# VITA-Group/CV_A-FAN

Hardware: AMD Instinct MI355X
Metric: images/sec (whole node) A-FAN K=5 train step, ResNet-18/CIFAR-10 (higher is better)
Workload: dtype bf16; 1 GPU; resnet18 CIFAR-10-shape A-FAN K=5 bf16, batch 256/GPU, perturb_idx 6, internal layout nhwc, 1xMI355X per rank (BASELINE configs[1]); global_batch=256, parallelism=dp1, hipgraph=True, in_launch_batchnorm=True

## Files before the change

cv_a-fan_amd/_lib.py:

```python
import ctypes as C
import os

_HERE = os.path.dirname(os.path.abspath(__file__))
LIB_PATH = os.environ.get("AFAN_HIP_LIB") or os.path.join(_HERE, "libafan_hip.so")

AFAN_F32, AFAN_BF16 = 0, 1
AFAN_NCHW, AFAN_NHWC = 0, 1
_ERRORS = {-1: "AFAN_EDTYPE (unknown dtype code)", -2: "AFAN_EALIGN (misaligned pointer)",
           -3: "AFAN_ESHAPE (bad sizes)", -4: "AFAN_ENULL (required pointer is NULL)",
           -5: "AFAN_ELAYOUT (unknown layout code)"}

_p, _i, _l, _f = C.c_void_p, C.c_int, C.c_int64, C.c_float

SIGNATURES = {
    "afan_version": (_i, []),
    "afan_arch": (C.c_char_p, []),
    "afan_pgd_step": (_i, [_p, _p, _i, _p, _p, _l, _f, _f, _i, _p]),
    "afan_tensor_clamp": (_i, [_p, _p, _p, _l, _p]),
    "afan_norms_workspace_floats": (_l, [_l, _l]),
    "afan_pgd_step_norms": (_i, [_p, _p, _i, _p, _p, _l, _l, _f, _f, _i, _p, _p, _p, _p]),
    "afan_perturb_norms": (_i, [_p, _p, _l, _l, _p, _p, _p, _p]),
    "afan_axpy_noise": (_i, [_p, _p, _l, _f, _p, _p]),
    "afan_mix_feature": (_i, [_p, _p, _p, _l, _l, _l, _f, _i, _p]),
    "afan_mix_feature_nhwc": (_i, [_p, _p, _p, _l, _l, _l, _f, _i, _p]),
    "afan_lerp_points": (_i, [_p, _p, _p, _l, C.POINTER(_f), _i, _p]),
    "afan_lerp_mix": (_i, [_p, _p, _p, _l, _l, _l, C.POINTER(_f), _i, C.c_uint, _f, _i, _p]),
    "afan_head_max_classes": (_i, []),
    "afan_head_forward": (_i, [_p, _i, _l, _l, _l, _p, _p, _l, _p, _p, _p]),
    "afan_head_backward": (_i, [_p, _p, _p, _l, _l, _l, _l, _p, _i, _p, _p, _i, _p]),
    "afan_cross_entropy": (_i, [_p, _p, _l, _l, _p, _p, _p]),
    "afan_mix_w_workspace_floats": (_l, []),
    "afan_mix_w": (_i, [_p, _p, _p, _p, _i, _l, _p]),
    "afan_mix_w_backward": (_i, [_p, _i, _p, _p, _l, _p, _p, _i, _p]),
    "afan_bn_workspace_floats": (_l, [_l]),
    "afan_bn_acc_doubles": (_l, [_l]),
    "afan_bn_acc_supported": (_i, [_i, _l]),
    "afan_bn_set_running_updates": (_i, [_i]),
    "afan_bn_running_update": (_i, [_p, _l, C.c_double, _f, _f, _p, _p, _p, _p]),
    "afan_bn_running_update_batched": (_i, [_p, _p, _p, _p, _p, _p, _p, _p, _i, _p]),
    "afan_bn_train_forward_acc": (_i, [_p, _p, _p, _i, _l, _l, _l, _f, _f, _p, _p, _i, _p, _i, _p, _p, _p, _p, _i, _p]),
    "afan_bn_train_forward_acc_dual": (_i, [_p, _p, _p, _i, _l, _l, _l, _f, _f, _p, _p, _p, _p, _p, _p, _p, _f, _f, _p, _p, _p, _p,
                                            _p, _p, _p, _p]),
    "afan_bn_backward_acc": (_i, [_p, _p, _p, _p, _p, _i, _l, _l, _l, _p, _i, _p, _i, _p, _p, _i, _i, _p]),
    "afan_bn_stats": (_i, [_p, _i, _i, _l, _l, _l, _f, _f, _p, _p, _p, _p, _p, _p]),
    "afan_bn_train_forward": (_i, [_p, _p, _p, _i, _i, _l, _l, _l, _f, _f, _p, _p, _i, _p, _p, _p, _p, _p, _p]),
    "afan_bn_apply": (_i, [_p, _p, _p, _i, _i, _l, _l, _l, _p, _p, _p, _p, _i, _p, _p]),
    "afan_bn_backward": (_i, [_p, _p, _p, _p, _p, _i, _i, _l, _l, _l, _p, _p, _p, _i, _p, _p, _p, _i, _p, _l, _p]),
    "afan_conv_supported": (_i, [_l, _l, _i, _i]),
    "afan_conv_fwd_nhwc_bf16": (_i, [_p, _p, _p, _l, _l, _l, _l, _l, _i, _i, _i, _p, _p, _p, _i, _p]),
    "afan_conv_fwd_affine_nhwc_bf16": (_i, [_p, _p, _p, _l, _l, _l, _l, _l, _i, _i, _p, _p, _i, _p]),
    "afan_conv_fwd_affine_any_nhwc_bf16": (_i, [_p, _p, _p, _l, _l, _l, _l, _l, _i, _i, _p, _p, _i, _p]),
    "afan_conv_fwd_multi_nhwc_bf16": (_i, [_p, _p, _p, _i, _l, _l, _l, _l, _l, _p, _i, _p, _p, _p, _i, _p]),
    "afan_conv_fwd_tiles": (_l, [_l, _l, _l, _l, _l, _i, _i]),
    "afan_bn_train_forward_partials": (_i, [_p, _p, _p, _i, _l, _l, _l, _f, _f, _p, _p, _i, _p, _l, _p, _p, _p, _p, _p, _p]),
    "afan_conv_dgrad_nhwc_bf16": (_i, [_p, _p, _p, _l, _l, _l, _l, _l, _i, _i, _i, _p, _p, _p, _i, _p, _p, _p, _i, _p]),
    "afan_conv_dgrad_affine_nhwc_bf16": (_i, [_p, _p, _p, _l, _l, _l, _l, _l, _i, _i, _p, _p, _p]),
    "afan_conv_dgrad_dual_nhwc_bf16": (_i, [_p, _p, _p, _p, _l, _l, _l, _l, _l, _i, _i, _p, _p, _p, _p]),
    "afan_conv_dgrad_sc_nhwc_bf16": (_i, [_p, _p, _p, _p, _l, _l, _l, _l, _l, _p, _p, _i, _p, _p, _p, _p]),
    "afan_grid_barrier_bytes": (_i, []),
    "afan_grid_barrier_error_word": (_i, []),
    "afan_grid_barrier_shared_gpu": (_i, [_i]),
    "afan_conv_fwd_bn_nhwc_bf16": (_i, [_p, _p, _p, _p, _l, _l, _l, _l, _l, _i, _i, _p, _p, _p, _p, _f, _f, _p, _p, _p, _p, _p, _i, _p, _p, _p, _p,
                                        _f, _f, _p, _p, _p, _p, _p, _p]),
    "afan_conv_dgrad_bn_nhwc_bf16": (_i, [_p, _p, _p, _p, _l, _l, _l, _l, _l, _i, _i, _p, _p, _p, _i, _p, _p, _p, _p, _i, _p, _p, _p, _p, _p, _p,
                                          _p, _p]),
    "afan_conv_fwd_multi_bn_nhwc_bf16": (_i, [_p, _p, _p, _i, _l, _l, _l, _l, _l, _p, _i, _p, _p, _p, _p, _p, _p, _f, _f, _p, _p, _p, _p, _i, _p,
                                              _p]),
    "afan_conv_dgrad_sc_bn_nhwc_bf16": (_i, [_p, _p, _p, _p, _p, _l, _l, _l, _l, _l, _p, _p, _i, _p, _p, _p, _p, _i, _p, _p]),
    "afan_conv_dgrad_tiles": (_l, [_l, _l, _l, _l, _l, _i, _i]),
    "afan_conv_wgrad_workspace_floats": (_l, [_l, _l, _l, _l, _l, _i, _i]),
    "afan_conv_wgrad_nhwc_bf16": (_i, [_p, _p, _p, _l, _l, _l, _l, _l, _i, _i, _i, _p, _i, _p]),
    "afan_conv_wgrad_plan": (_i, [_l, _l, _l, _l, _l, _i, _i]),
    "afan_conv_wgrad_multi_nhwc_bf16": (_i, [_i, _p, _p, _p, _p, _p, _p, _p, _p, _p, _p, _p, _p, _i, _p]),
    "afan_conv_wgrad2_nhwc_bf16": (_i, [_p, _p, _l, _p, _p, _l, _p, _l, _l, _l, _l, _i, _i, _i, _p, _i, _p]),
    "afan_conv_fwd": (_i, [_p, _p, _p, _p, _i, _i, _i, _l, _l, _l, _l, _l, _i, _i, _i, _i, _p]),
    "afan_conv_dgrad": (_i, [_p, _p, _p, _i, _i, _i, _l, _l, _l, _l, _l, _i, _i, _i, _i, _p]),
    "afan_conv_wgrad_f32_workspace_floats": (_l, [_l, _l, _l, _l, _l, _i, _i, _i, _i]),
    "afan_conv_wgrad": (_i, [_p, _p, _p, _i, _i, _i, _l, _l, _l, _l, _l, _i, _i, _i, _i, _p, _i, _p]),
    "afan_conv_stem7_supported": (_i, [_l, _l, _i, _i]),
    "afan_conv_stem7_fwd_nhwc_bf16": (_i, [_p, _p, _p, _l, _l, _l, _p]),
    "afan_conv_stem7_im2col_k": (_i, []),
    "afan_conv_stem7_im2col": (_i, [_p, _p, _l, _l, _l, _p]),
    "afan_conv_stem7_col2im": (_i, [_p, _p, _l, _l, _l, _p]),
    "afan_conv_stem7_wgrad_workspace_floats": (_l, [_l, _l, _l]),
    "afan_conv_stem7_wgrad_nhwc_bf16": (_i, [_p, _p, _p, _l, _l, _l, _p, _i, _p]),
    "afan_upsample_bilinear_fwd": (_i, [_p, _p, _i, _i, _l, _l, _l, _l, _l, _l, _p]),
    "afan_upsample_bilinear_bwd": (_i, [_p, _p, _i, _i, _l, _l, _l, _l, _l, _l, _p]),
    "afan_upsample_bilinear_fwd_slice": (_i, [_p, _p, _i, _l, _l, _l, _l, _l, _l, _l, _p]),
    "afan_upsample_bilinear_bwd_workspace_floats": (_l, [_l, _l, _l, _l]),
    "afan_upsample_bilinear_bwd_slice": (_i, [_p, _p, _i, _l, _l, _l, _l, _l, _l, _l, _p, _p]),
    "afan_ce2d_workspace_floats": (_l, [_l]),
    "afan_ce2d": (_i, [_p, _p, _i, _l, _l, _l, _l, _f, _p, _p, _p, _p]),
    "afan_ce2d_upsampled_workspace_floats": (_l, [_l, _l, _l, _l, _l, _l]),
    "afan_ce2d_upsampled": (_i, [_p, _p, _l, _l, _l, _l, _l, _l, _l, _f, _p, _p, _p, _p]),
    "afan_maxpool3x3s2_fwd": (_i, [_p, _p, _i, _i, _l, _l, _l, _l, _p]),
    "afan_maxpool3x3s2_bwd": (_i, [_p, _p, _p, _i, _i, _l, _l, _l, _l, _p]),
    "afan_maxpool2d_fwd": (_i, [_p, _p, _p, _i, _i, _l, _l, _l, _l, _i, _i, _i, _p]),
    "afan_maxpool2d_bwd": (_i, [_p, _p, _p, _p, _i, _i, _l, _l, _l, _l, _i, _i, _i, _p]),
    "afan_affine_relu_bwd": (_i, [_p, _p, _p, _p, _p, _i, _i, _l, _l, _l, _i, _p]),
    "afan_affine_coefs": (_i, [_p, _p, _p, _p, _l, _p, _p]),
    "afan_frozen_bottleneck_fwd": (_i, [_p, _l, _l, _l, _l, _l, _i, _p, _p, _p, _p, _p, _p, _p, _p, _p, _p, _p, _p, _p]),
    "afan_frozen_bottleneck_bwd_scratch": (_l, [_l, _l, _l, _l, _l, _i]),
    "afan_frozen_bottleneck_bwd": (_i, [_p, _p, _p, _p, _p, _l, _l, _l, _l, _l, _i, _p, _p, _p, _p, _p, _p, _p, _p, _p, _p, _p, _p, _p, _p,
                                        _p, _p]),
    "afan_frozen_bottleneck_bwd_chain": (_i, [_p, _p, _p, _p, _p, _p, _p, _l, _l, _l, _l, _l, _i, _p, _p, _p, _p, _p, _p, _p, _p, _p, _p, _p, _p, _p,
                                              _p, _p, _p, _p, _p, _p]),
    "afan_affine_apply": (_i, [_p, _p, _p, _i, _l, _l, _l, _p, _i, _p]),
    "afan_avgpool_fwd": (_i, [_p, _p, _i, _i, _l, _l, _l, _i, _p]),
    "afan_avgpool_bwd": (_i, [_p, _p, _i, _i, _l, _l, _l, _i, _p]),
    "afan_linear_small_max_rows": (_i, []),
    "afan_linear_small_fwd": (_i, [_p, _p, _p, _l, _l, _l, _p]),
    "afan_linear_small_bwd": (_i, [_p, _p, _p, _p, _p, _l, _l, _l, _i, _p]),
    "afan_pointwise_max_co": (_i, []),
    "afan_pointwise_fwd": (_i, [_p, _i, _p, _p, _p, _l, _l, _l, _p]),
    "afan_pointwise_bwd_dx": (_i, [_p, _p, _p, _i, _l, _l, _l, _p]),
    "afan_pointwise_workspace_floats": (_l, [_l, _l, _l]),
    "afan_pointwise_bwd_dw": (_i, [_p, _p, _i, _p, _p, _l, _l, _l, _p, _i, _p]),
    "afan_dropout": (_i, [_p, _p, _i, _l, _f, _p, _p, _p, _i, _p]),
    "afan_nms_workspace_bytes": (_l, [_l]),
    "afan_nms": (_i, [_p, _p, _l, _f, _i, _p, _p, _p, _p]),
    "afan_nms_top": (_i, [_p, _p, _l, _f, _i, _p, _p, _p, _l, _p]),
    "afan_box_decode_clip": (_i, [_p, _p, _p, _l, _f, _f, _p]),
    "afan_box_assign": (_i, [_p, _p, _l, _l, _l, _i, _f, _f, _p, _p, _p, _p, _p]),
    "afan_sample_lists": (_i, [_p, _l, _p, _p, _p, _p]),
    "afan_sample_gather": (_i, [_p, _p, _p, _l, _p, _p, _p, _p, _l, _l, _p, _p, _p, _p, _p, _p]),
    "afan_det_loss_fwd": (_i, [_p, _p, _p, _p, _p, _p, _l, _l, _l, _l, _f, _p, _p, _p, _p, _p]),
    "afan_sum_scalars_f32": (_i, [_p, _p, _p, _p, _p, _p]),
    "afan_linear_pair_workspace_floats": (_l, [_i, _l, _l, _l, _l]),
    "afan_linear_pair_fwd_f32": (_i, [_p, _p, _p, _p, _p, _p, _p, _l, _l, _l, _l, _p, _p]),
    "afan_linear_pair_dgrad_f32": (_i, [_p, _p, _p, _p, _p, _l, _l, _l, _l, _p]),
    "afan_linear_pair_wgrad_f32": (_i, [_p, _p, _p, _p, _p, _p, _p, _i, _l, _l, _l, _l, _p, _p]),
    "afan_proposal_rows": (_i, [_p, _l, _p, _l, _p, _l, _p, _p, _p]),
    "afan_labels_limit": (_i, [_p, _l, _l, _p, _l, _p]),
    "afan_det_loss_bwd": (_i, [_p, _p, _p, _p, _p, _p, _l, _l, _l, _l, _l, _p, _p, _p]),
    "afan_roi_align_fwd": (_i, [_p, _p, _p, _i, _i, _l, _l, _l, _l, _i, _i, _f, _i, _p]),
    "afan_roi_align_bwd": (_i, [_p, _p, _p, _i, _i, _l, _l, _l, _l, _l, _i, _i, _f, _i, _p]),
    "afan_roi_align_bwd_workspace_bytes": (_l, [_l, _l, _l]),
    "afan_roi_align_bwd_ws": (_i, [_p, _p, _p, _i, _i, _l, _l, _l, _l, _l, _i, _i, _f, _i, _p, _p]),
    "afan_transpose_weights": (_i, [_p, _p, _p, _i, _l, _p]),
    "afan_sgd_step": (_i, [_p, _p, _p, _p, _l, _p, _f, _f, _f, _i, _p]),
    "afan_sgd_step_guarded": (_i, [_p, _p, _p, _p, _l, _p, _f, _f, _f, _i, _p, _p]),
    "afan_guarded_copy": (_i, [_p, _p, _l, _p, _p, _p]),
    "afan_occupy_cus": (_i, [_i, _i, _i, _p]),
    "afan_cast_bf16": (_i, [_p, _p, _l, _p]),
    "afan_pgd_init": (_i, [_p, _i, _p, _p, _p, _l, _p]),
    "afan_normalize_nchw": (_i, [_p, _p, _i, _i, _l, _l, _l, _p, _p, _p]),
    "afan_profile_enable": (_i, [_i]),
    "afan_profile_collect": (_i, [C.c_char_p, C.POINTER(_l), C.POINTER(C.c_double), C.POINTER(C.c_double),
                                  C.POINTER(C.c_double), _i]),
    "afan_profile_event_overhead": (_i, [_i, C.POINTER(_f), _p]),
    "afan_conv_trace": (_i, [_i]),
    "afan_conv_trace_read": (_i, [C.POINTER(_l), C.c_char_p, _i]),
}

_lib = None


class AfanLibraryError(RuntimeError):
    pass


def load():
    global _lib
    if _lib is not None:
        return _lib
    if not os.path.exists(LIB_PATH):
        raise AfanLibraryError(
            f"{LIB_PATH} is missing: build it with `python -c 'import __graft_entry__ as g; g.build()'` "
            "(or `make -C cv_a-fan_amd/csrc`). There is no CPU or PyTorch fallback for the A-FAN kernels.")
    lib = C.CDLL(LIB_PATH)
    for name, (res, args) in SIGNATURES.items():
        fn = getattr(lib, name)
        fn.restype = res
        fn.argtypes = args
    _lib = lib
    return lib


def check(rc, what):
    if rc == 0:
        return
    if rc < 0:
        raise AfanLibraryError(f"{what}: {_ERRORS.get(rc, rc)}")
    raise AfanLibraryError(f"{what}: HIP launch failed with hipError_t={rc}")
```

cv_a-fan_amd/attack_algo.py:

```python
import torch

from . import ops
from .resnet_s import _dense, _like_layout, dgrad_only, fused_criterion

__all__ = ["PGD", "tensor_clamp", "linfball_proj", "mix_feature", "get_sample_points", "last_norms"]

_last = {"l2": None, "linf": None}


def last_norms():
    return _last["l2"], _last["linf"]


def tensor_clamp(t, min, max, in_place=True):
    res = t if in_place else t.clone()
    ops.tensor_clamp_(res.data, min.contiguous(), max.contiguous())
    return res


def linfball_proj(center, radius, t, in_place=True):
    res = t if in_place else t.clone()
    zero = torch.zeros_like(res.data)
    ops.pgd_step_(res.data, zero, 0.0, x_clean=center.contiguous(), eps=float(radius), clip=True)
    return res


def PGD(x, loss_fn, y=None, model=None, steps=3, gamma=None, start_idx=1, layer_number=16, eps=(2 / 255),
        randinit=False, clip=False, with_norms=False, grad0=None):
    if x.device.type != "cuda":
        raise ops.AfanLibraryError("PGD: x must live on the MI355X (no CPU path in this build)")
    lp = getattr(model, "compute_dtype", torch.float32) == torch.bfloat16
    if grad0 is not None and (randinit or steps < 1):
        raise ValueError("grad0 is the gradient at x: not with randinit, and only when there is a first step")
    x, x_adv, shadow = ops.pgd_init(_dense(x.detach()), want_shadow=lp and grad0 is None and not randinit)
    if lp and shadow is None:
        shadow = torch.empty_like(x, dtype=torch.bfloat16)
    if randinit:
        u = _like_layout(torch.rand(x_adv.shape).to(x.device, non_blocking=True), x_adv)
        ops.axpy_noise_(x_adv, u, eps, shadow)
    l2 = linf = None
    loss_fn = fused_criterion(loss_fn, model)
    for t in range(steps):
        if t == 0 and grad0 is not None:
            grad = grad0.detach()
        else:
            xin = (shadow if lp else x_adv).detach().requires_grad_(True)
            with dgrad_only():
                out = model(xin, end_point=layer_number, start_point=start_idx)
                loss = loss_fn(out, y)
                root = ops.one(loss.device) if (loss.dim() == 0 and loss.dtype == torch.float32) else None
                grad = torch.autograd.grad(loss, xin, grad_outputs=root, only_inputs=True)[0]
        grad = _like_layout(grad, x_adv)
        if with_norms and t == steps - 1:
            l2, linf = ops.pgd_step_norms_(x_adv, grad, gamma, x, eps, clip, shadow)
        else:
            ops.pgd_step_(x_adv, grad, gamma, x, eps, clip, shadow)
    if with_norms:
        if l2 is None:
            l2, linf = ops.perturb_norms(x_adv, x)
        _last["l2"], _last["linf"] = l2, linf
    x_adv.requires_grad_(True)
    if lp:
        x_adv._afan_shadow = shadow
    return x_adv


def mix_feature(clean_feature, adv_feature):
    return ops.mix_feature(_dense(clean_feature), _dense(adv_feature), 1e-5)


def sample_points_mixed(pointx, pointy, number, mix):
    px, py = _dense(pointx), _dense(pointy)
    if py.stride() != px.stride():
        py = _like_layout(py, px)
    return [pointx] + ops.lerp_mix(px, py, number, [bool(f) for f in mix])


def get_sample_points(pointx, pointy, number):
    px, py = _dense(pointx), _dense(pointy)
    if py.stride() != px.stride():
        py = _like_layout(py, px)
    inner = ops.lerp_points(px, py, number)
    return [pointx] + inner + [pointy]
```

cv_a-fan_amd/csrc/afan_head.hip:

```cpp
#include "afan_common.h"

using namespace afan;

namespace {

constexpr int BLOCK = 256;
constexpr int MAXK = 16;

template <typename T>
__global__ __launch_bounds__(BLOCK) void head_fwd_kernel(const T* __restrict__ x, const float* __restrict__ W,
                                                         const float* __restrict__ bias, float* __restrict__ pooled,
                                                         float* __restrict__ logits, int C, int HW, int K) {
    const int b = blockIdx.x;
    const T* xb = x + (int64_t)b * HW * C;
    float part[MAXK];
#pragma unroll
    for (int k = 0; k < MAXK; ++k) part[k] = 0.f;
    const float inv = 1.0f / (float)HW;
    for (int c = threadIdx.x; c < C; c += BLOCK) {
        float s = 0.f;
        for (int p = 0; p < HW; ++p) s += Elt<T>::ld(xb + (int64_t)p * C + c);
        const float m = s * inv;
        pooled[(int64_t)b * C + c] = m;
#pragma unroll
// ... 15 lines not shown
}

__global__ __launch_bounds__(BLOCK) void head_fwd_vec_kernel(const uint16_t* __restrict__ x, const float* __restrict__ W,
                                                             const float* __restrict__ bias, float* __restrict__ pooled,
                                                             float* __restrict__ logits, int C, int HW, int K) {
    __shared__ float grp[BLOCK * 8];
    __shared__ float red[BLOCK / AFAN_WAVE][MAXK];
    const int b = blockIdx.x, P = C >> 3, G = BLOCK / P;
    const int pc = threadIdx.x % P, pg = threadIdx.x / P;
    const uint16_t* xb = x + (int64_t)b * HW * C + pc * 8;
    float s[8];
#pragma unroll
    for (int j = 0; j < 8; ++j) s[j] = 0.f;
    for (int p = pg; p < HW; p += G) {
        const u16x8 v = *reinterpret_cast<const u16x8*>(xb + (int64_t)p * C);
#pragma unroll
        for (int j = 0; j < 8; ++j) s[j] += bf2f(v[j]);
    }
#pragma unroll
    for (int j = 0; j < 8; ++j) grp[pg * C + pc * 8 + j] = s[j];
    __syncthreads();
    float part[MAXK];
#pragma unroll
    for (int k = 0; k < MAXK; ++k) part[k] = 0.f;
    const float inv = 1.0f / (float)HW;
    for (int c = threadIdx.x; c < C; c += BLOCK) {
        float t = 0.f;
        for (int g = 0; g < G; ++g) t += grp[g * C + c];
        const float m = t * inv;
        pooled[(int64_t)b * C + c] = m;
#pragma unroll
        for (int k = 0; k < MAXK; ++k)
            if (k < K) part[k] = fmaf(m, W[(int64_t)k * C + c], part[k]);
    }
#pragma unroll
    for (int k = 0; k < MAXK; ++k) {
        const float v = wave_sum(part[k]);
        if ((threadIdx.x & 63) == 0) red[threadIdx.x >> 6][k] = v;
    }
    __syncthreads();
    if (threadIdx.x < K) {
        float t = bias ? bias[threadIdx.x] : 0.f;
        for (int w = 0; w < BLOCK / AFAN_WAVE; ++w) t += red[w][threadIdx.x];
        logits[(int64_t)b * K + threadIdx.x] = t;
    }
}

template <typename T>
__global__ __launch_bounds__(BLOCK) void head_bwd_dx_kernel(const float* __restrict__ dlogits, const float* __restrict__ W,
                                                            T* __restrict__ dx, int C, int HW, int K) {
    const int b = blockIdx.x;
    __shared__ float dl[MAXK];
    if (threadIdx.x < K) dl[threadIdx.x] = dlogits[(int64_t)b * K + threadIdx.x];
    __syncthreads();
    const float inv = 1.0f / (float)HW;
    T* xb = dx + (int64_t)b * HW * C;
    for (int c = threadIdx.x; c < C; c += BLOCK) {
        float g = 0.f;
        for (int k = 0; k < K; ++k) g = fmaf(dl[k], W[(int64_t)k * C + c], g);
        g *= inv;
        for (int p = 0; p < HW; ++p) Elt<T>::st(xb + (int64_t)p * C + c, g);
    }
}

constexpr int DW_SLICES = 16;
__global__ __launch_bounds__(64 * DW_SLICES) void head_bwd_dw_kernel(const float* __restrict__ dlogits,
                                                                    const float* __restrict__ pooled, float* __restrict__ dW,
                                                                    float* __restrict__ db, int B, int C, int K, int accumulate) {
    __shared__ float red[DW_SLICES][64];
    const int e = threadIdx.x & 63, q = threadIdx.x >> 6;
    const int64_t i = (int64_t)blockIdx.x * 64 + e;
    const int64_t KC = (int64_t)K * C, total = KC + (db ? K : 0);
    float s = 0.f;
    if (i < KC) {
        const int k = (int)(i / C), c = (int)(i % C);
        for (int b = q; b < B; b += DW_SLICES) s = fmaf(dlogits[(int64_t)b * K + k], pooled[(int64_t)b * C + c], s);
    } else if (i < total) {
        const int k = (int)(i - KC);
        for (int b = q; b < B; b += DW_SLICES) s += dlogits[(int64_t)b * K + k];
    }
    red[q][e] = s;
    __syncthreads();
    if (q == 0 && i < total) {
        float sum = 0.f;
#pragma unroll
        for (int j = 0; j < DW_SLICES; ++j) sum += red[j][e];
        float* dst = i < KC ? dW + i : db + (i - KC);
        *dst = accumulate ? *dst + sum : sum;
    }
}

constexpr int CE_BLOCK = 256;
__global__ __launch_bounds__(CE_BLOCK) void ce_fwd_kernel(const float* __restrict__ logits, const int64_t* __restrict__ target,
                                                          float* __restrict__ loss, float* __restrict__ dlogits, int N, int K) {
    __shared__ float red[CE_BLOCK / AFAN_WAVE];
    const float invn = 1.0f / (float)N;
    float local = 0.f;
    for (int r = threadIdx.x; r < N; r += CE_BLOCK) {
        const float* l = logits + (int64_t)r * K;
        float m = l[0];
        for (int k = 1; k < K; ++k) m = fmaxf(m, l[k]);
        float s = 0.f;
        for (int k = 0; k < K; ++k) s += expf(l[k] - m);
        const float lse = m + logf(s);
        const int64_t t64 = target[r];
        const bool bad = t64 < 0 || t64 >= K;
        const int t = bad ? 0 : (int)t64;
        local += bad ? NAN : lse - l[t];
        float* d = dlogits + (int64_t)r * K;
        for (int k = 0; k < K; ++k) d[k] = bad ? NAN : (expf(l[k] - lse) - (k == t ? 1.f : 0.f)) * invn;
    }
    const float w = wave_sum(local);
    if ((threadIdx.x & 63) == 0) red[threadIdx.x >> 6] = w;
    __syncthreads();
    if (threadIdx.x == 0) {
        float s = 0.f;
        for (int i = 0; i < CE_BLOCK / AFAN_WAVE; ++i) s += red[i];
        loss[0] = s * invn;
    }
}

constexpr int CEW_WAVES = 16;
__global__ __launch_bounds__(64 * CEW_WAVES) void ce_fwd_wide_kernel(const float* __restrict__ logits, const int64_t* __restrict__ target,
                                                                     float* __restrict__ loss, float* __restrict__ dlogits, int N, int K) {
    __shared__ float red[CEW_WAVES];
    const int lane = threadIdx.x & 63, w = threadIdx.x >> 6;
    const float invn = 1.0f / (float)N;
    float local = 0.f;
    for (int r = w; r < N; r += CEW_WAVES) {
        const float* l = logits + (int64_t)r * K;
        float m = -INFINITY;
        for (int k = lane; k < K; k += 64) m = fmaxf(m, l[k]);
        m = wave_max(m);
        float s = 0.f;
        for (int k = lane; k < K; k += 64) s += expf(l[k] - m);
        s = wave_sum(s);
        const float lse = m + logf(s);
        const int64_t t64 = target[r];
        const bool bad = t64 < 0 || t64 >= K;
        const int t = bad ? 0 : (int)t64;
        if (lane == 0) local += bad ? NAN : lse - l[t];
        float* d = dlogits + (int64_t)r * K;
        for (int k = lane; k < K; k += 64) d[k] = bad ? NAN : (expf(l[k] - lse) - (k == t ? 1.f : 0.f)) * invn;
    }
    if (lane == 0) red[w] = local;
    __syncthreads();
    if (threadIdx.x == 0) {
        float s = 0.f;
        for (int i = 0; i < CEW_WAVES; ++i) s += red[i];
        loss[0] = s * invn;
    }
}

}

extern "C" {

int afan_head_max_classes(void) { return MAXK; }

int afan_head_forward(const void* x, int dtype, int64_t n, int64_t c, int64_t hw, const float* weight, const float* bias,
                      int64_t k, float* pooled, float* logits, afan_stream_t stream) {
    if (dtype != AFAN_F32 && dtype != AFAN_BF16) return AFAN_EDTYPE;
    if (n <= 0 || c <= 0 || hw <= 0 || k <= 0 || k > MAXK) return AFAN_ESHAPE;
    if (!x || !weight || !pooled || !logits) return AFAN_ENULL;
    hipStream_t st = (hipStream_t)stream;
    AFAN_PROF("head_fwd_kernel", (double)n * hw * c * (dtype == AFAN_F32 ? 4 : 2), st);
    if (dtype == AFAN_F32)
        head_fwd_kernel<float><<<(unsigned)n, BLOCK, 0, st>>>((const float*)x, weight, bias, pooled, logits, (int)c, (int)hw, (int)k);
    else if (c % 8 == 0 && c / 8 <= BLOCK && BLOCK % (c / 8) == 0 && aligned(x, 16))
        head_fwd_vec_kernel<<<(unsigned)n, BLOCK, 0, st>>>((const uint16_t*)x, weight, bias, pooled, logits, (int)c, (int)hw, (int)k);
    else
        head_fwd_kernel<uint16_t><<<(unsigned)n, BLOCK, 0, st>>>((const uint16_t*)x, weight, bias, pooled, logits, (int)c, (int)hw, (int)k);
    AFAN_LAUNCH_CHECK();
    return AFAN_OK;
}

int afan_head_backward(const float* dlogits, const float* weight, const float* pooled, int64_t n, int64_t c, int64_t hw,
                       int64_t k, void* dx, int dx_dtype, float* dweight, float* dbias, int accumulate,
                       afan_stream_t stream) {
    if (dx && dx_dtype != AFAN_F32 && dx_dtype != AFAN_BF16) return AFAN_EDTYPE;
    if (n <= 0 || c <= 0 || hw <= 0 || k <= 0 || k > MAXK) return AFAN_ESHAPE;
    if (!dlogits || !weight || !pooled) return AFAN_ENULL;
    hipStream_t st = (hipStream_t)stream;
    if (dx) {
        AFAN_PROF("head_bwd_dx_kernel", (double)n * hw * c * (dx_dtype == AFAN_F32 ? 4 : 2), st);
        if (dx_dtype == AFAN_F32)
            head_bwd_dx_kernel<float><<<(unsigned)n, BLOCK, 0, st>>>(dlogits, weight, (float*)dx, (int)c, (int)hw, (int)k);
        else
            head_bwd_dx_kernel<uint16_t><<<(unsigned)n, BLOCK, 0, st>>>(dlogits, weight, (uint16_t*)dx, (int)c, (int)hw, (int)k);
        AFAN_LAUNCH_CHECK();
    }
    if (dweight) {
        AFAN_PROF("head_bwd_dw_kernel", 4.0 * n * (c + k), st);
        const unsigned grid = (unsigned)((k * c + (dbias ? k : 0) + 63) / 64);
        head_bwd_dw_kernel<<<grid, 64 * DW_SLICES, 0, st>>>(dlogits, pooled, dweight, dbias, (int)n, (int)c, (int)k, accumulate);
        AFAN_LAUNCH_CHECK();
    }
    return AFAN_OK;
}

int afan_cross_entropy(const float* logits, const int64_t* target, int64_t n, int64_t k, float* loss, float* dlogits,
                       afan_stream_t stream) {
    if (n <= 0 || k <= 0 || n * k > (1 << 16)) return AFAN_ESHAPE;
    if (!logits || !target || !loss || !dlogits) return AFAN_ENULL;
    hipStream_t st = (hipStream_t)stream;
    AFAN_PROF("ce_fwd_kernel", 8.0 * n * k, st);
    if (k >= 64) ce_fwd_wide_kernel<<<1, 64 * CEW_WAVES, 0, st>>>(logits, target, loss, dlogits, (int)n, (int)k);
    else ce_fwd_kernel<<<1, CE_BLOCK, 0, st>>>(logits, target, loss, dlogits, (int)n, (int)k);
    AFAN_LAUNCH_CHECK();
    return AFAN_OK;
}

}
```

cv_a-fan_amd/csrc/afan_pgd.hip:

```cpp
#include "afan_common.h"

using namespace afan;

namespace {

constexpr int BLOCK = 256;
constexpr int NORM_CHUNK = 4096;

__device__ __forceinline__ float sign_of(float g) {
    return (g != g) ? g : (float)((g > 0.f) - (g < 0.f));
}

template <bool CLIP>
__device__ __forceinline__ float step_one(float xa, float g, float xc, float gamma, float eps) {
    float d = gamma * sign_of(g);
    float t = xa + d;
    if (CLIP) {
        float lo = xc - eps;
        float hi = xc + eps;
        if (t < lo) t = lo;
        if (t > hi) t = hi;
    }
    return t;
}
// ... 111 lines not shown
                }
            }
#pragma unroll
            for (int k = 0; k < 4; ++k) {
                float d = xa[k] - xc[k];
                ss += d * d;
                mx = absmax_nan(mx, d);
            }
        }
    } else {
        for (int64_t j = lo + threadIdx.x; j < hi; j += BLOCK) {
            const int64_t i = base + j;
            float xa = x_adv[i], xc = x_clean[i];
            if (STEP) {
                xa = step_one<CLIP>(xa, Elt<G>::ld(grad + i), xc, gamma, eps);
                x_adv[i] = xa;
                if (SHADOW) shadow[i] = f2bf(xa);
            }
            float d = xa - xc;
            ss += d * d;
            mx = absmax_nan(mx, d);
        }
    }
    block_reduce_store(ss, mx, partial, b * gridDim.x + blockIdx.x);
}

__global__ __launch_bounds__(AFAN_WAVE) void norms_finalize_kernel(const float* __restrict__ partial,
                                                                   int slices, float* __restrict__ l2,
                                                                   float* __restrict__ linf) {
    const int64_t b = blockIdx.x;
    float ss = 0.f, mx = 0.f;
    for (int s = threadIdx.x; s < slices; s += AFAN_WAVE) {
        ss += partial[2 * (b * slices + s)];
        float m = partial[2 * (b * slices + s) + 1];
        mx = (m != m || mx != mx) ? __builtin_nanf("") : fmaxf(mx, m);
    }
    ss = wave_sum(ss);
    float isn = (mx != mx) ? 1.f : 0.f;
    isn = wave_max(isn);
    mx = wave_max((mx != mx) ? 0.f : mx);
    if (threadIdx.x == 0) {
        l2[b] = sqrtf(ss);
        linf[b] = (isn > 0.f) ? __builtin_nanf("") : mx;
    }
}

__global__ __launch_bounds__(BLOCK) void axpy_noise_kernel(float* __restrict__ x_adv,
                                                           const float* __restrict__ u, int64_t n,
                                                           float eps, uint16_t* __restrict__ shadow,
                                                           int vec) {
    const int64_t tid = (int64_t)blockIdx.x * BLOCK + threadIdx.x;
    const int64_t nthreads = (int64_t)gridDim.x * BLOCK;
    int64_t done = 0;
    if (vec) {
        const int64_t nvec = n >> 2;
        for (int64_t v = tid; v < nvec; v += nthreads) {
            const int64_t i = v << 2;
            float xa[4], uu[4];
            Elt<float>::ldv(x_adv + i, xa);
            Elt<float>::ldv(u + i, uu);
#pragma unroll
            for (int k = 0; k < 4; ++k) {
                float t = 2.0f * uu[k];
                t = t - 1.0f;
                t = t * eps;
                xa[k] = xa[k] + t;
            }
            Elt<float>::stv(x_adv + i, xa);
            if (shadow) {
                u16x4 s;
#pragma unroll
                for (int k = 0; k < 4; ++k) s[k] = f2bf(xa[k]);
                *reinterpret_cast<u16x4*>(shadow + i) = s;
            }
        }
        done = nvec << 2;
    }
    for (int64_t i = done + tid; i < n; i += nthreads) {
        float t = 2.0f * u[i];
        t = t - 1.0f;
        t = t * eps;
        t = x_adv[i] + t;
        x_adv[i] = t;
        if (shadow) shadow[i] = f2bf(t);
    }
}

__global__ __launch_bounds__(BLOCK) void tensor_clamp_kernel(float* __restrict__ t, const float* __restrict__ lo,
                                                             const float* __restrict__ hi, int64_t n) {
    for (int64_t i = (int64_t)blockIdx.x * BLOCK + threadIdx.x; i < n; i += (int64_t)gridDim.x * BLOCK) {
        float v = t[i];
        const float l = lo[i], h = hi[i];
        if (v < l) v = l;
        if (v > h) v = h;
        t[i] = v;
    }
}

__global__ __launch_bounds__(BLOCK) void cast_bf16_kernel(const float* __restrict__ src,
                                                          uint16_t* __restrict__ dst, int64_t n, int vec) {
    const int64_t tid = (int64_t)blockIdx.x * BLOCK + threadIdx.x;
    const int64_t nthreads = (int64_t)gridDim.x * BLOCK;
    int64_t done = 0;
    if (vec) {
        const int64_t nvec = n >> 3;
        for (int64_t v = tid; v < nvec; v += nthreads) {
            const int64_t i = v << 3;
            float a[4], b[4];
            Elt<float>::ldv(src + i, a);
            Elt<float>::ldv(src + i + 4, b);
            float o[8] = {a[0], a[1], a[2], a[3], b[0], b[1], b[2], b[3]};
            Elt<uint16_t>::stv(dst + i, o);
        }
        done = nvec << 3;
    }
    for (int64_t i = done + tid; i < n; i += nthreads) dst[i] = f2bf(src[i]);
}


template <typename S>
__global__ __launch_bounds__(BLOCK) void pgd_init_kernel(const S* __restrict__ x, float* __restrict__ x32,
                                                         float* __restrict__ x_adv, uint16_t* __restrict__ shadow, int64_t n, int vec) {
    const int64_t tid = (int64_t)blockIdx.x * BLOCK + threadIdx.x;
    const int64_t nthreads = (int64_t)gridDim.x * BLOCK;
    int64_t done = 0;
    if (vec) {
        const int64_t nvec = n >> 3;
        for (int64_t v = tid; v < nvec; v += nthreads) {
            const int64_t i = v << 3;
            float o[8];
            if constexpr (sizeof(S) == 4) {
                float a[4], b[4];
                Elt<float>::ldv((const float*)x + i, a);
                Elt<float>::ldv((const float*)x + i + 4, b);
#pragma unroll
                for (int e = 0; e < 4; ++e) { o[e] = a[e]; o[4 + e] = b[e]; }
            } else {
                Elt<uint16_t>::ldv((const uint16_t*)x + i, o);
            }
            const float lo[4] = {o[0], o[1], o[2], o[3]}, hi[4] = {o[4], o[5], o[6], o[7]};
            if (x32) { Elt<float>::stv(x32 + i, lo); Elt<float>::stv(x32 + i + 4, hi); }
            Elt<float>::stv(x_adv + i, lo);
            Elt<float>::stv(x_adv + i + 4, hi);
            if (shadow) Elt<uint16_t>::stv(shadow + i, o);
        }
        done = nvec << 3;
    }
    for (int64_t i = done + tid; i < n; i += nthreads) {
        const float v = Elt<S>::ld(x + i);
        if (x32) x32[i] = v;
        x_adv[i] = v;
        if (shadow) shadow[i] = f2bf(v);
    }
}

template <typename G, bool CLIP, bool SHADOW>
int launch_step(float* x_adv, const void* grad, const float* x_clean, uint16_t* shadow, int64_t n,
                float gamma, float eps, hipStream_t st) {
    const bool vec = aligned(x_adv, 16) && aligned(grad, 4 * sizeof(G)) &&
                     (!CLIP || aligned(x_clean, 16)) && (!SHADOW || aligned(shadow, 8));
    const int grid = grid_for(vec ? (n + 3) / 4 : n, BLOCK);
    AFAN_PROF("pgd_step_kernel", n * (8.0 + sizeof(G) + (CLIP ? 4 : 0) + (SHADOW ? 2 : 0)), st);
    if (vec)
        pgd_step_kernel<G, CLIP, SHADOW, true><<<grid, BLOCK, 0, st>>>(
            x_adv, (const G*)grad, x_clean, shadow, n, gamma, eps);
    else
        pgd_step_kernel<G, CLIP, SHADOW, false><<<grid, BLOCK, 0, st>>>(
            x_adv, (const G*)grad, x_clean, shadow, n, gamma, eps);
    AFAN_LAUNCH_CHECK();
    return AFAN_OK;
}

template <typename G, bool CLIP, bool SHADOW, bool STEP>
int launch_step_norms(float* x_adv, const void* grad, const float* x_clean, uint16_t* shadow,
                      int64_t batch, int64_t per_sample, float gamma, float eps, float* partial,
                      float* l2, float* linf, hipStream_t st) {
    const bool vec = (per_sample % 4 == 0) && aligned(x_adv, 16) && aligned(x_clean, 16) &&
                     (!STEP || aligned(grad, 4 * sizeof(G))) && (!SHADOW || aligned(shadow, 8));
    const int slices = (int)((per_sample + NORM_CHUNK - 1) / NORM_CHUNK);
    dim3 grid(slices, (unsigned)batch);
    {
        const double elts = (double)batch * (double)per_sample;
        AFAN_PROF(STEP ? "pgd_step_norms_kernel" : "perturb_norms_kernel",
                  elts * (STEP ? (12.0 + sizeof(G) + (SHADOW ? 2 : 0)) : 8.0), st);
        if (vec)
            pgd_step_norms_kernel<G, CLIP, SHADOW, true, STEP><<<grid, BLOCK, 0, st>>>(
                x_adv, (const G*)grad, x_clean, shadow, per_sample, gamma, eps, partial);
        else
            pgd_step_norms_kernel<G, CLIP, SHADOW, false, STEP><<<grid, BLOCK, 0, st>>>(
                x_adv, (const G*)grad, x_clean, shadow, per_sample, gamma, eps, partial);
    }
    AFAN_LAUNCH_CHECK();
    AFAN_PROF("norms_finalize_kernel", 8.0 * batch * slices, st);
    norms_finalize_kernel<<<(unsigned)batch, AFAN_WAVE, 0, st>>>(partial, slices, l2, linf);
    AFAN_LAUNCH_CHECK();
    return AFAN_OK;
}

}

extern "C" {

int afan_version(void) { return 100; }
const char* afan_arch(void) { return "gfx950"; }

int afan_pgd_step(float* x_adv, const void* grad, int grad_dtype, const float* x_clean,
                  uint16_t* shadow_bf16, int64_t n, float gamma, float eps, int clip,
                  afan_stream_t stream) {
    if (n < 0) return AFAN_ESHAPE;
    if (n == 0) return AFAN_OK;
    if (!x_adv || !grad || (clip && !x_clean)) return AFAN_ENULL;
    if (grad_dtype != AFAN_F32 && grad_dtype != AFAN_BF16) return AFAN_EDTYPE;
    if (!aligned(x_adv, 4) || !aligned(grad, grad_dtype == AFAN_F32 ? 4 : 2) ||
        (clip && !aligned(x_clean, 4)) || (shadow_bf16 && !aligned(shadow_bf16, 2)))
        return AFAN_EALIGN;
    hipStream_t st = (hipStream_t)stream;
#define AFAN_DISPATCH(G)                                                                              \
    if (clip) {                                                                                       \
        if (shadow_bf16) return launch_step<G, true, true>(x_adv, grad, x_clean, shadow_bf16, n, gamma, eps, st); \
        return launch_step<G, true, false>(x_adv, grad, x_clean, shadow_bf16, n, gamma, eps, st);     \
    } else {                                                                                          \
        if (shadow_bf16) return launch_step<G, false, true>(x_adv, grad, x_clean, shadow_bf16, n, gamma, eps, st); \
        return launch_step<G, false, false>(x_adv, grad, x_clean, shadow_bf16, n, gamma, eps, st);    \
    }
    if (grad_dtype == AFAN_F32) { AFAN_DISPATCH(float) }
    AFAN_DISPATCH(uint16_t)
#undef AFAN_DISPATCH
}

int64_t afan_norms_workspace_floats(int64_t batch, int64_t per_sample) {
    if (batch <= 0 || per_sample <= 0) return 0;
    return 2 * batch * ((per_sample + NORM_CHUNK - 1) / NORM_CHUNK);
}

int afan_pgd_step_norms(float* x_adv, const void* grad, int grad_dtype, const float* x_clean,
                        uint16_t* shadow_bf16, int64_t batch, int64_t per_sample, float gamma,
                        float eps, int clip, float* partial, float* l2_out, float* linf_out,
                        afan_stream_t stream) {
    if (batch < 0 || per_sample <= 0 || batch > 65535) return AFAN_ESHAPE;
    if (batch == 0) return AFAN_OK;
    if (!x_adv || !grad || !x_clean || !partial || !l2_out || !linf_out) return AFAN_ENULL;
    if (grad_dtype != AFAN_F32 && grad_dtype != AFAN_BF16) return AFAN_EDTYPE;
    if (!aligned(x_adv, 4) || !aligned(grad, grad_dtype == AFAN_F32 ? 4 : 2) || !aligned(x_clean, 4) ||
        !aligned(partial, 4) || (shadow_bf16 && !aligned(shadow_bf16, 2)))
        return AFAN_EALIGN;
    hipStream_t st = (hipStream_t)stream;
#define AFAN_DISPATCH(G)                                                                             \
    if (clip) {                                                                                      \
        if (shadow_bf16)                                                                             \
            return launch_step_norms<G, true, true, true>(x_adv, grad, x_clean, shadow_bf16, batch,  \
                                                          per_sample, gamma, eps, partial, l2_out, linf_out, st); \
        return launch_step_norms<G, true, false, true>(x_adv, grad, x_clean, shadow_bf16, batch,     \
                                                       per_sample, gamma, eps, partial, l2_out, linf_out, st); \
    } else {                                                                                         \
        if (shadow_bf16)                                                                             \
            return launch_step_norms<G, false, true, true>(x_adv, grad, x_clean, shadow_bf16, batch, \
                                                           per_sample, gamma, eps, partial, l2_out, linf_out, st); \
        return launch_step_norms<G, false, false, true>(x_adv, grad, x_clean, shadow_bf16, batch,    \
                                                        per_sample, gamma, eps, partial, l2_out, linf_out, st); \
    }
    if (grad_dtype == AFAN_F32) { AFAN_DISPATCH(float) }
    AFAN_DISPATCH(uint16_t)
#undef AFAN_DISPATCH
}

int afan_perturb_norms(const float* x_adv, const float* x_clean, int64_t batch, int64_t per_sample,
                       float* partial, float* l2_out, float* linf_out, afan_stream_t stream) {
    if (batch < 0 || per_sample <= 0 || batch > 65535) return AFAN_ESHAPE;
    if (batch == 0) return AFAN_OK;
    if (!x_adv || !x_clean || !partial || !l2_out || !linf_out) return AFAN_ENULL;
    if (!aligned(x_adv, 4) || !aligned(x_clean, 4) || !aligned(partial, 4)) return AFAN_EALIGN;
    return launch_step_norms<float, false, false, false>(const_cast<float*>(x_adv), nullptr, x_clean,
                                                         nullptr, batch, per_sample, 0.f, 0.f, partial,
                                                         l2_out, linf_out, (hipStream_t)stream);
}

int afan_axpy_noise(float* x_adv, const float* u, int64_t n, float eps, uint16_t* shadow_bf16,
                    afan_stream_t stream) {
    if (n < 0) return AFAN_ESHAPE;
    if (n == 0) return AFAN_OK;
    if (!x_adv || !u) return AFAN_ENULL;
    if (!aligned(x_adv, 4) || !aligned(u, 4) || (shadow_bf16 && !aligned(shadow_bf16, 2))) return AFAN_EALIGN;
    const int vec = aligned(x_adv, 16) && aligned(u, 16) && (!shadow_bf16 || aligned(shadow_bf16, 8));
    const int grid = grid_for(vec ? (n + 3) / 4 : n, BLOCK);
    AFAN_PROF("axpy_noise_kernel", n * (12.0 + (shadow_bf16 ? 2 : 0)), (hipStream_t)stream);
    axpy_noise_kernel<<<grid, BLOCK, 0, (hipStream_t)stream>>>(x_adv, u, n, eps, shadow_bf16, vec);
    AFAN_LAUNCH_CHECK();
    return AFAN_OK;
}

int afan_tensor_clamp(float* t, const float* lo, const float* hi, int64_t n, afan_stream_t stream) {
    if (n < 0) return AFAN_ESHAPE;
    if (n == 0) return AFAN_OK;
    if (!t || !lo || !hi) return AFAN_ENULL;
    if (!aligned(t, 4) || !aligned(lo, 4) || !aligned(hi, 4)) return AFAN_EALIGN;
    AFAN_PROF("tensor_clamp_kernel", n * 16.0, (hipStream_t)stream);
    tensor_clamp_kernel<<<grid_for(n, BLOCK), BLOCK, 0, (hipStream_t)stream>>>(t, lo, hi, n);
    AFAN_LAUNCH_CHECK();
    return AFAN_OK;
}

int afan_cast_bf16(const float* src, uint16_t* dst, int64_t n, afan_stream_t stream) {
    if (n < 0) return AFAN_ESHAPE;
    if (n == 0) return AFAN_OK;
    if (!src || !dst) return AFAN_ENULL;
    if (!aligned(src, 4) || !aligned(dst, 2)) return AFAN_EALIGN;
    const int vec = aligned(src, 16) && aligned(dst, 16);
    const int grid = grid_for(vec ? (n + 7) / 8 : n, BLOCK);
    AFAN_PROF("cast_bf16_kernel", n * 6.0, (hipStream_t)stream);
    cast_bf16_kernel<<<grid, BLOCK, 0, (hipStream_t)stream>>>(src, dst, n, vec);
    AFAN_LAUNCH_CHECK();
    return AFAN_OK;
}

int afan_pgd_init(const void* x, int dtype, float* x32, float* x_adv, uint16_t* shadow, int64_t n, afan_stream_t stream) {
    if (dtype != AFAN_F32 && dtype != AFAN_BF16) return AFAN_EDTYPE;
    if (n < 0) return AFAN_ESHAPE;
    if (n == 0) return AFAN_OK;
    if (!x || !x_adv || (dtype == AFAN_BF16 && !x32)) return AFAN_ENULL;
    const size_t a = dtype == AFAN_F32 ? 4 : 2;
    if (!aligned(x, a) || !aligned(x_adv, 4) || (x32 && !aligned(x32, 4)) || (shadow && !aligned(shadow, 2))) return AFAN_EALIGN;
    hipStream_t st = (hipStream_t)stream;
    const int vec = aligned(x, 16) && aligned(x_adv, 16) && (!x32 || aligned(x32, 16)) && (!shadow || aligned(shadow, 16));
    const int grid = grid_for(vec ? (n + 7) / 8 : n, BLOCK);
    AFAN_PROF("pgd_init_kernel", n * (a + 4.0 + (x32 ? 4 : 0) + (shadow ? 2 : 0)), st);
    if (dtype == AFAN_F32) pgd_init_kernel<float><<<grid, BLOCK, 0, st>>>((const float*)x, x32, x_adv, shadow, n, vec);
    else pgd_init_kernel<uint16_t><<<grid, BLOCK, 0, st>>>((const uint16_t*)x, x32, x_adv, shadow, n, vec);
    AFAN_LAUNCH_CHECK();
    return AFAN_OK;
}

}
```

cv_a-fan_amd/learnable.py:

```python
import torch

from .grid_guard import GuardedTrainer

from . import ops
from .arena import ArenaSGD, ParamArena
from .attack_algo import PGD
from . import resnet_s
from .resnet_s import _like_layout

LEARNABLE_IDX = (4, 8, 11, 14, 18, 21, 24, 28, 31)


def sum_project(b, K=9):
    return b - (torch.sum(b, dim=0) - 1) / K


class _MixW(torch.autograd.Function):

    @staticmethod
    def forward(ctx, w, idx, clean, adv, out_dtype):
        ctx.save_for_backward(clean, adv)
        ctx.idx, ctx.nw = idx, w.numel()
        return ops.mix_w(clean, adv, w.detach()[idx:idx + 1], out_dtype)

    @staticmethod
    def backward(ctx, g):
        clean, adv = ctx.saved_tensors
        dw = torch.zeros(ctx.nw, dtype=torch.float32, device=clean.device)
        ops.mix_w_backward(_like_layout(g, clean), clean, adv, dw[ctx.idx:ctx.idx + 1])
        return dw, None, None, None, None


class LearnableTrainer(GuardedTrainer):

    def __init__(self, model, criterion, *, steps=3, gamma=1.0, eps=2.0, idx_list=LEARNABLE_IDX, layer_number=None,
                 randinit=False, clip=False, lr=0.1, w_lr=0.01, l1_coef=1.0, momentum=0.9, weight_decay=5e-4,
                 use_graph=True, graph_warmup=3):
        self.model, self.criterion = model, criterion
        self.steps, self.gamma, self.eps = steps, gamma, eps
        self.idx_list = tuple(idx_list)
        self.layer_number = layer_number if layer_number is not None else model.layer_number
        if len(self.idx_list) != model.w.numel():
            raise ValueError("one mixing weight per perturbed depth")
        self.randinit, self.clip, self.l1_coef = randinit, clip, l1_coef
        self.arena = ParamArena(model, index_root=getattr(model, "sequential_model", None))
        self.optimizer = ArenaSGD(self.arena, lr, momentum, weight_decay)
        self.optimizer_w = torch.optim.SGD([{"params": model.w, "lr": w_lr, "weight_decay": 0}], w_lr,
                                           momentum=momentum, weight_decay=0)
        self.use_graph = bool(use_graph) and not randinit
        self.graph_warmup = graph_warmup
        self._graph = self._graph_failed = self._static = self._out = self._key = None
        self._eager_steps = 0
        self._guard_init(model, self.arena.param.device)

    def _guard_state(self):
        st = self.optimizer_w.state.get(self.model.w, {})
        mb = st.get("momentum_buffer")
        return (self.model.w.detach().clone(), None if mb is None else mb.clone())

    def _guard_restore(self, state):
        w, mb = state
        with torch.no_grad():
            self.model.w.copy_(w)
        st = self.optimizer_w.state.get(self.model.w)
        if st is not None:
            if mb is None:
                st.pop("momentum_buffer", None)
            else:
                st["momentum_buffer"].copy_(mb)

    def _drop_graphs(self):
        self._graph = self._graph_failed = self._static = self._out = self._key = None

    def step(self, inp, target):
        return self._guarded((inp, target), self._step_once)

    def _step_once(self, inp, target):
        key = (tuple(inp.shape), inp.dtype, tuple(target.shape))
        if self._graph is not None and self._key == key:
            return self._replay(inp, target)
        if (self.use_graph and self._graph is None and self._graph_failed is None and inp.is_cuda
                and self._eager_steps >= self.graph_warmup and self.model.training and self._graph_safe()):
            try:
                self._capture(inp, target, key)
                return self._replay(inp, target)
            except Exception as e:
                import warnings
                self._graph, self._graph_failed = None, e
                warnings.warn(f"hipGraph capture of the learnable A-FAN step failed ({type(e).__name__}: {e}); running eagerly")
                torch.cuda.synchronize()
        self._eager_steps += 1
        self.optimizer._sync_lr()
        return self._body(inp, target)

    def _graph_safe(self):
        if resnet_s.vendor_convs(self.model):
            self.use_graph = False
        return self.use_graph

    def _capture(self, inp, target, key):
        dev = inp.device
        self._static = (torch.empty_like(inp), torch.empty_like(target))
        self._static[0].copy_(inp)
        self._static[1].copy_(target)
        stream = torch.cuda.Stream(device=dev)
        stream.wait_stream(torch.cuda.current_stream(dev))
        torch.cuda.synchronize(dev)
        g = torch.cuda.CUDAGraph()
        with ops.no_gc_during_capture(), torch.cuda.graph(g, stream=stream, capture_error_mode="thread_local"):
            out = self._body(self._static[0], self._static[1])
        self._graph, self._out, self._key = g, out, key

    def _replay(self, inp, target):
        self._static[0].copy_(inp, non_blocking=True)
        self._static[1].copy_(target, non_blocking=True)
        self.optimizer._sync_lr()
        self._graph.replay()
        return {k: v.clone() for k, v in self._out.items() if k != "out_clean"} | {"out_clean": self._out["out_clean"]}

    def _body(self, inp, target):
        m, ln = self.model, self.layer_number
        if inp.is_cuda:
            ops.acc_reset(inp.device)
        clean, adv = [], []
        for num in self.idx_list:
            with torch.no_grad():
                fea = m(inp, end_point=num, start_point=0)
            fea = fea.float() if fea.dtype != torch.float32 else fea
            clean.append(fea)
            adv.append(PGD(fea, self.criterion, y=target, model=m, steps=self.steps, gamma=(self.gamma / 255),
                           start_idx=num, layer_number=ln, eps=(self.eps / 255), randinit=self.randinit,
                           clip=self.clip))
        dtype = getattr(m, "compute_dtype", torch.float32)
        outs, l2s, linfs = [], [], []
        for i, num in enumerate(self.idx_list):
            l2, linf = ops.perturb_norms(adv[i].detach(), clean[i])
            l2s.append(l2)
            linfs.append(linf)
            mixed = _MixW.apply(m.w, i, clean[i], adv[i].detach(), dtype)
            outs.append(m(mixed, end_point=ln, start_point=num))
        out_clean = m(inp, end_point=ln, start_point=0)
        loss_adv = 0
        for o in outs:
            loss_adv = loss_adv + self.criterion(o.float(), target)
        loss_clean = self.criterion(out_clean.float(), target)
        l1 = torch.norm(m.w, p=1)
        loss = (loss_clean + loss_adv / len(self.idx_list)) / 2 + l1 * self.l1_coef
        self.optimizer.zero_grad()
        self.optimizer_w.zero_grad()
        loss.backward()
        self.optimizer.step()
        self.optimizer_w.step()
        with torch.no_grad():
            m.w.data.copy_(sum_project(m.w.data, K=len(self.idx_list)))
        prec1 = (out_clean.argmax(dim=1) == target).float().sum() * (100.0 / target.shape[0])
        return {"loss": loss.detach(), "loss_clean": loss_clean.detach(), "loss_adv": loss_adv.detach(),
                "l1": l1.detach(), "l2": torch.stack(l2s), "linf": torch.stack(linfs), "prec1": prec1,
                "w": m.w.detach().clone(), "out_clean": out_clean.detach()}
```

cv_a-fan_amd/ops.py:

```python
import ctypes as C
import os
import threading

import torch

from . import _lib
from ._lib import AFAN_BF16, AFAN_F32, AFAN_NCHW, AFAN_NHWC, AfanLibraryError, check

_DT = {torch.float32: AFAN_F32, torch.bfloat16: AFAN_BF16}
_ws_cache = {}
_tls = threading.local()
CALLS = {"conv_fwd": 0, "conv_dgrad": 0, "conv_wgrad": 0, "conv_general": 0, "vendor_conv": 0, "conv_bn_fused": 0}


def _need(t, name, dtype=None):
    if not isinstance(t, torch.Tensor):
        raise TypeError(f"{name}: expected a torch.Tensor")
    if t.device.type != "cuda":
        raise AfanLibraryError(f"{name}: tensor is on '{t.device}'. The A-FAN kernels are MI355X-only; "
                               "there is no CPU path (the CPU restatement under oracle/ is test infrastructure).")
    if not _dense(t):
        raise ValueError(f"{name}: tensor must be dense (contiguous NCHW or channels_last)")
    if dtype is not None and t.dtype != dtype:
        raise TypeError(f"{name}: expected {dtype}, got {t.dtype}")
# ... 144 lines not shown

def cross_entropy(logits, target):
    lib = _lib.load()
    _need(logits, "logits", torch.float32)
    if logits.dim() != 2 or not logits.is_contiguous() or target.dtype != torch.int64 or target.dim() != 1 \
            or target.shape[0] != logits.shape[0] or not target.is_cuda:
        raise TypeError("cross_entropy: logits [N,K] fp32 contiguous and target [N] int64 on the GPU")
    loss = torch.empty(1, dtype=torch.float32, device=logits.device)
    dlogits = torch.empty_like(logits)
    check(lib.afan_cross_entropy(_ptr(logits), _ptr(target.contiguous()), logits.shape[0], logits.shape[1], _ptr(loss),
                                 _ptr(dlogits), _stream(logits)), "afan_cross_entropy")
    return loss, dlogits


CE_MAX_ELEMS = 1 << 16
_ones = {}


def half(device):
    t = _ones.get(("half", device.index))
    if t is None:
        t = _ones[("half", device.index)] = torch.full((), 0.5, dtype=torch.float32, device=device)
    return t


def one(device):
    t = _ones.get(device.index)
    if t is None:
        t = _ones[device.index] = torch.ones((), dtype=torch.float32, device=device)
    return t


class bn_running_updates:

    def __init__(self, n):
        self.n = int(n)

    def __enter__(self):
        self.old = _lib.load().afan_bn_set_running_updates(self.n)
        return self

    def __exit__(self, *exc):
        _lib.load().afan_bn_set_running_updates(self.old)
        return False


def pgd_step_(x_adv, grad, gamma, x_clean=None, eps=0.0, clip=False, shadow=None):
    lib = _lib.load()
    _need(x_adv, "x_adv", torch.float32)
    _need(grad, "grad")
    if grad.dtype not in _DT or grad.numel() != x_adv.numel():
        raise TypeError("grad must be fp32/bf16 with x_adv's number of elements")
    if clip:
        _need(x_clean, "x_clean", torch.float32)
        if x_clean.numel() != x_adv.numel():
            raise ValueError("x_clean must match x_adv")
    if shadow is not None:
        _need(shadow, "shadow", torch.bfloat16)
    _same_layout(x_adv, grad, x_clean if clip else None, shadow)
    check(lib.afan_pgd_step(_ptr(x_adv), _ptr(grad), _DT[grad.dtype], _ptr(x_clean) if clip else None,
                            _ptr(shadow), x_adv.numel(), float(gamma), float(eps), int(bool(clip)),
                            _stream(x_adv)), "afan_pgd_step")
    return x_adv


def tensor_clamp_(t, lo, hi):
    lib = _lib.load()
    _need(t, "t", torch.float32)
    _need(lo, "min", torch.float32)
    _need(hi, "max", torch.float32)
    if lo.numel() != t.numel() or hi.numel() != t.numel():
        raise ValueError("min/max must match t")
    check(lib.afan_tensor_clamp(_ptr(t), _ptr(lo), _ptr(hi), t.numel(), _stream(t)), "afan_tensor_clamp")
    return t


def pgd_step_norms_(x_adv, grad, gamma, x_clean, eps=0.0, clip=False, shadow=None):
    lib = _lib.load()
    _need(x_adv, "x_adv", torch.float32)
    _need(grad, "grad")
    _need(x_clean, "x_clean", torch.float32)
    if grad.dtype not in _DT or grad.numel() != x_adv.numel() or x_clean.numel() != x_adv.numel():
        raise TypeError("grad/x_clean must match x_adv")
    if shadow is not None:
        _need(shadow, "shadow", torch.bfloat16)
    _same_layout(x_adv, grad, x_clean, shadow)
    batch = x_adv.shape[0]
    per = x_adv.numel() // max(batch, 1)
    out = torch.empty(2, batch, dtype=torch.float32, device=x_adv.device)
    if batch == 0:
        return out[0], out[1]
    ws = _workspace(x_adv, lib.afan_norms_workspace_floats(batch, per), "norms")
    check(lib.afan_pgd_step_norms(_ptr(x_adv), _ptr(grad), _DT[grad.dtype], _ptr(x_clean), _ptr(shadow),
                                  batch, per, float(gamma), float(eps), int(bool(clip)), _ptr(ws),
                                  _ptr(out[0]), _ptr(out[1]), _stream(x_adv)), "afan_pgd_step_norms")
    return out[0], out[1]


def perturb_norms(x_adv, x_clean):
    lib = _lib.load()
    _need(x_adv, "x_adv", torch.float32)
    _need(x_clean, "x_clean", torch.float32)
    if x_clean.numel() != x_adv.numel():
        raise ValueError("x_clean must match x_adv")
    _same_layout(x_adv, x_clean)
    batch = x_adv.shape[0]
    per = x_adv.numel() // max(batch, 1)
    out = torch.empty(2, batch, dtype=torch.float32, device=x_adv.device)
    if batch == 0:
        return out[0], out[1]
    ws = _workspace(x_adv, lib.afan_norms_workspace_floats(batch, per), "norms")
    check(lib.afan_perturb_norms(_ptr(x_adv), _ptr(x_clean), batch, per, _ptr(ws), _ptr(out[0]),
                                 _ptr(out[1]), _stream(x_adv)), "afan_perturb_norms")
    return out[0], out[1]


def axpy_noise_(x_adv, u, eps, shadow=None):
    lib = _lib.load()
    _need(x_adv, "x_adv", torch.float32)
    _need(u, "u", torch.float32)
    if u.numel() != x_adv.numel():
        raise ValueError("u must match x_adv")
    if shadow is not None:
        _need(shadow, "shadow", torch.bfloat16)
    _same_layout(x_adv, shadow)
    if u.shape == x_adv.shape and u.stride() != x_adv.stride():
        u = u.contiguous(memory_format=torch.channels_last) if layout_of(x_adv) == AFAN_NHWC else u.contiguous()
    check(lib.afan_axpy_noise(_ptr(x_adv), _ptr(u), x_adv.numel(), float(eps), _ptr(shadow),
                              _stream(x_adv)), "afan_axpy_noise")
    return x_adv


def cast_bf16(src, out=None):
    lib = _lib.load()
    _need(src, "src", torch.float32)
    if out is None:
        out = torch.empty_like(src, dtype=torch.bfloat16)
    _need(out, "out", torch.bfloat16)
    _same_layout(src, out)
    check(lib.afan_cast_bf16(_ptr(src), _ptr(out), src.numel(), _stream(src)), "afan_cast_bf16")
    return out


def pgd_init(x, want_shadow=False):
    lib = _lib.load()
    _need(x, "x")
    if x.dtype not in _DT:
        raise TypeError("x must be fp32 or bf16")
    x32 = x if x.dtype == torch.float32 else torch.empty_like(x, dtype=torch.float32)
    x_adv = torch.empty_like(x, dtype=torch.float32)
    shadow = torch.empty_like(x, dtype=torch.bfloat16) if want_shadow else None
    check(lib.afan_pgd_init(_ptr(x), _DT[x.dtype], None if x32 is x else _ptr(x32), _ptr(x_adv),
                            None if shadow is None else _ptr(shadow), x.numel(), _stream(x)), "afan_pgd_init")
    return x32, x_adv, shadow


def mix_feature(clean, adv, eps=1e-5):
    lib = _lib.load()
    _need(clean, "clean")
    _need(adv, "adv", clean.dtype)
    if clean.dtype not in _DT or clean.shape != adv.shape:
        raise TypeError("clean/adv must be fp32 or bf16 tensors of the same shape")
    if layout_of(clean) != layout_of(adv):
        adv = adv.contiguous(memory_format=torch.channels_last if layout_of(clean) == AFAN_NHWC else torch.contiguous_format)
    n, c, hw = _nchw(clean)
    out = torch.empty_like(clean)
    fn = lib.afan_mix_feature_nhwc if layout_of(clean) == AFAN_NHWC else lib.afan_mix_feature
    check(fn(_ptr(clean), _ptr(adv), _ptr(out), n, c, hw, float(eps), _DT[clean.dtype], _stream(clean)),
          "afan_mix_feature")
    return out


def lerp_points(x, y, number):
    lib = _lib.load()
    _need(x, "x", torch.float32)
    _need(y, "y", torch.float32)
    if x.shape != y.shape:
        raise ValueError("x/y shape mismatch")
    _same_layout(x, y)
    k = number - 2
    if k <= 0:
        return []
    if k > 8:
        raise ValueError("at most 10 sample points")
    percent = 1.0 / (number - 1)
    w = (C.c_float * k)(*[i * percent for i in range(1, number - 1)])
    flat = torch.empty(k * x.numel(), dtype=torch.float32, device=x.device)
    out = [flat[i * x.numel():(i + 1) * x.numel()].as_strided(x.shape, x.stride()) for i in range(k)]
    check(lib.afan_lerp_points(_ptr(x), _ptr(y), _ptr(flat), x.numel(), w, k, _stream(x)), "afan_lerp_points")
    return out


def lerp_mix(x, y, number, mix, eps=1e-5):
    lib = _lib.load()
    _need(x, "x", torch.float32)
    _need(y, "y", torch.float32)
    if x.shape != y.shape or x.dim() != 4:
        raise ValueError("x/y must be 4-d tensors of the same shape")
    _same_layout(x, y)
    npts = number - 1
    if npts < 1 or npts > 4 or len(mix) != npts:
        raise ValueError("2..5 sample points, one mix flag per point after the first")
    n, c, hw = _nchw(x)
    percent = 1.0 / (number - 1)
    w = (C.c_float * max(npts - 1, 1))(*[i * percent for i in range(1, number - 1)])
    mask = sum(1 << j for j, f in enumerate(mix) if f)
    flat = torch.empty(npts * x.numel(), dtype=torch.float32, device=x.device)
    out = [flat[i * x.numel():(i + 1) * x.numel()].as_strided(x.shape, x.stride()) for i in range(npts)]
    check(lib.afan_lerp_mix(_ptr(x), _ptr(y), _ptr(flat), n, c, hw, w, number, mask, float(eps), layout_of(x), _stream(x)),
          "afan_lerp_mix")
    if not mix[-1]:
        out[-1] = y
    return out


def mix_w(clean, adv, w_elem, out_dtype=torch.float32):
    lib = _lib.load()
    _need(clean, "clean", torch.float32), _need(adv, "adv", torch.float32), _need(w_elem, "w", torch.float32)
    _same_layout(clean, adv)
    if w_elem.numel() != 1 or out_dtype not in _DT:
        raise ValueError("w must be a single fp32 element; out_dtype fp32 or bf16")
    out = torch.empty_like(clean, dtype=out_dtype)
    check(lib.afan_mix_w(_ptr(clean), _ptr(adv), _ptr(w_elem), _ptr(out), _DT[out_dtype], clean.numel(),
                         _stream(clean)), "afan_mix_w")
    return out


def mix_w_backward(grad_out, clean, adv, dw_elem, accumulate=False):
    lib = _lib.load()
    _need(grad_out, "grad_out"), _need(clean, "clean", torch.float32), _need(adv, "adv", torch.float32)
    _need(dw_elem, "dw", torch.float32)
    _same_layout(clean, adv, grad_out)
    if grad_out.dtype not in _DT or dw_elem.numel() != 1:
        raise TypeError("grad_out must be fp32 or bf16, dw a single fp32 element")
    ws = _workspace(clean, lib.afan_mix_w_workspace_floats(), "mixw")
    check(lib.afan_mix_w_backward(_ptr(grad_out), _DT[grad_out.dtype], _ptr(clean), _ptr(adv), clean.numel(), _ptr(ws),
                                  _ptr(dw_elem), int(bool(accumulate)), _stream(clean)), "afan_mix_w_backward")
    return dw_elem


def head_forward(x, weight, bias):
    lib = _lib.load()
    _need(x, "x"), _need(weight, "weight", torch.float32)
    if x.dim() != 4 or not (layout_of(x) == AFAN_NHWC or x.shape[2] * x.shape[3] == 1) or x.dtype not in _DT:
        raise ValueError("head_forward: x must be a channels-last fp32/bf16 feature map")
    n, c, hw = _nchw(x)
    k = weight.shape[0]
    pooled = torch.empty(n, c, dtype=torch.float32, device=x.device)
    logits = torch.empty(n, k, dtype=torch.float32, device=x.device)
    check(lib.afan_head_forward(_ptr(x), _DT[x.dtype], n, c, hw, _ptr(weight), _ptr(bias), k, _ptr(pooled), _ptr(logits),
                                _stream(x)), "afan_head_forward")
    return logits, pooled


def head_backward(dlogits, weight, pooled, x_like, want_dx, dweight=None, dbias=None, accumulate=False):
    lib = _lib.load()
    _need(dlogits, "dlogits", torch.float32), _need(pooled, "pooled", torch.float32)
    n, c, hw = _nchw(x_like)
    dx = torch.empty_like(x_like) if want_dx else None
    check(lib.afan_head_backward(_ptr(dlogits.contiguous()), _ptr(weight), _ptr(pooled), n, c, hw, weight.shape[0], _ptr(dx),
                                 _DT[x_like.dtype], _ptr(dweight), _ptr(dbias), int(bool(accumulate)), _stream(x_like)),
          "afan_head_backward")
    return dx


def bn_stats(x, eps=1e-5, momentum=0.1, running_mean=None, running_var=None, num_batches=None):
    lib = _lib.load()
    _need(x, "x")
    n, c, hw = _nchw(x)
    stats = torch.empty(4, c, dtype=torch.float32, device=x.device)
    ws = _workspace(x, lib.afan_bn_workspace_floats(c), "bn")
    check(lib.afan_bn_stats(_ptr(x), _DT[x.dtype], layout_of(x), n, c, hw, float(eps), float(momentum), _ptr(ws),
                            _ptr(stats), _ptr(running_mean), _ptr(running_var), _ptr(num_batches), _stream(x)),
          "afan_bn_stats")
    return stats[0], stats[1]


class record_bn_updates:

    def __enter__(self):
        self.old = getattr(_tls, "bn_rec", None)
        self.items = _tls.bn_rec = []
        return self

    def __exit__(self, *exc):
        _tls.bn_rec = self.old
        return False

    def replay(self):
        lib = _lib.load()
        it = self.items
        n = len(it)
        if n == 0:
            return
        ptrs = lambda k: (C.c_void_p * n)(*[(t[k].data_ptr() if t[k] is not None else None) for t in it])
        check(lib.afan_bn_running_update_batched(
            ptrs(3), ptrs(0), ptrs(1), ptrs(2), (C.c_int64 * n)(*[t[0].numel() for t in it]),
            (C.c_double * n)(*[float(t[4]) for t in it]), (C.c_float * n)(*[float(t[5]) for t in it]),
            (C.c_float * n)(*[float(t[6]) for t in it]), n, _stream(it[0][0])), "afan_bn_running_update_batched")


def _bn_record(running_mean, running_var, num_batches, stats, m, eps, momentum, groups):
    rec = getattr(_tls, "bn_rec", None)
    if rec is not None and running_mean is not None:
        if groups != 1:
            raise ValueError("record_bn_updates: grouped BatchNorm launches cannot be replayed")
        rec.append((running_mean, running_var, num_batches, stats, m, eps, momentum))


def bn_train_forward(x, weight, bias, residual, relu, eps, momentum, running_mean, running_var, num_batches,
                     conv_stats=None, out=None, stats_out=None, groups=1):
    lib = _lib.load()
    _need(x, "x")
    if x.dtype not in _DT:
        raise TypeError("x must be fp32 or bf16")
    if residual is not None:
        _need(residual, "residual", x.dtype)
        _same_layout(x, residual)
    n, c, hw = _nchw(x)
    if out is not None:
        _need(out, "out", x.dtype)
        _same_layout(x, out)
    y = out if out is not None else torch.empty_like(x)
    if groups != 1 and (conv_stats is None or conv_stats.acc is None):
        raise ValueError("grouped BatchNorm needs the accumulators of a grouped convolution")
    stats = stats_out if stats_out is not None else torch.empty((4, c) if groups == 1 else (groups, 4, c),
                                                                dtype=torch.float32, device=x.device)
    _bn_record(running_mean, running_var, num_batches, stats, n * hw, eps, momentum, groups)
    acc = conv_stats.acc if conv_stats is not None else None
    ready = acc is not None
    if acc is None and conv_stats is None and bn_acc_ok(x):
        acc = acc_take(x.device, c)
    if acc is not None:
        if layout_of(x) != AFAN_NHWC and not (x.shape[2] == 1 and x.shape[3] == 1):
            raise ValueError("accumulator statistics need a channels_last x")
        check(lib.afan_bn_train_forward_acc(_ptr(x), _ptr(residual), _ptr(y), _DT[x.dtype], n, c, hw, float(eps),
                                            float(momentum), _ptr(weight), _ptr(bias), int(bool(relu)), _ptr(acc),
                                            int(ready), _ptr(stats), _ptr(running_mean), _ptr(running_var),
                                            _ptr(num_batches), int(groups), _stream(x)), "afan_bn_train_forward_acc")
        return y, stats
    if conv_stats is not None:
        if layout_of(x) != AFAN_NHWC and not (x.shape[2] == 1 and x.shape[3] == 1):
            raise ValueError("conv_stats need a channels_last x")
        check(lib.afan_bn_train_forward_partials(_ptr(x), _ptr(residual), _ptr(y), _DT[x.dtype], n, c, hw, float(eps),
                                                 float(momentum), _ptr(weight), _ptr(bias), int(bool(relu)),
                                                 _ptr(conv_stats.partials), int(conv_stats.g), _ptr(conv_stats.shift),
                                                 _ptr(stats), _ptr(running_mean), _ptr(running_var), _ptr(num_batches),
                                                 _stream(x)), "afan_bn_train_forward_partials")
        return y, stats
    ws = _workspace(x, lib.afan_bn_workspace_floats(c), "bn")
    check(lib.afan_bn_train_forward(_ptr(x), _ptr(residual), _ptr(y), _DT[x.dtype], layout_of(x), n, c, hw, float(eps),
                                    float(momentum), _ptr(weight), _ptr(bias), int(bool(relu)), _ptr(ws), _ptr(stats),
                                    _ptr(running_mean), _ptr(running_var), _ptr(num_batches), _stream(x)),
          "afan_bn_train_forward")
    return y, stats


def bn_train_forward_dual(xa, bna, sta, mom_a, xb, bnb, stb, mom_b):
    lib = _lib.load()
    _need(xa, "xa"), _need(xb, "xb", xa.dtype)
    _same_layout(xa, xb)
    n, c, hw = _nchw(xa)
    y = torch.empty_like(xa)
    stats = torch.empty((2, 4, c), dtype=torch.float32, device=xa.device)
    _bn_record(bnb.running_mean, bnb.running_var, bnb.num_batches_tracked, stats[1], n * hw, bnb.eps, mom_b, 1)
    _bn_record(bna.running_mean, bna.running_var, bna.num_batches_tracked, stats[0], n * hw, bna.eps, mom_a, 1)
    check(lib.afan_bn_train_forward_acc_dual(
        _ptr(xa), _ptr(xb), _ptr(y), _DT[xa.dtype], n, c, hw,
        float(bna.eps), float(mom_a), _ptr(bna.weight), _ptr(bna.bias), _ptr(sta.acc), _ptr(stats[0]), _ptr(bna.running_mean),
        _ptr(bna.running_var), _ptr(bna.num_batches_tracked),
        float(bnb.eps), float(mom_b), _ptr(bnb.weight), _ptr(bnb.bias), _ptr(stb.acc), _ptr(stats[1]), _ptr(bnb.running_mean),
        _ptr(bnb.running_var), _ptr(bnb.num_batches_tracked), _stream(xa)), "afan_bn_train_forward_acc_dual")
    return y, stats[0], stats[1]


def frozen_bottleneck_fwd(x, planes, stride, ws, ks):
    lib = _lib.load()
    _cl4(x, "x")
    n, cin, h, w = x.shape
    ho, wo = (h - 1) // stride + 1, (w - 1) // stride + 1
    co = 4 * planes
    cl = torch.channels_last
    a1 = torch.empty((n, planes, h, w), dtype=torch.bfloat16, device=x.device, memory_format=cl)
    a2 = torch.empty((n, planes, ho, wo), dtype=torch.bfloat16, device=x.device, memory_format=cl)
    out = torch.empty((n, co, ho, wo), dtype=torch.bfloat16, device=x.device, memory_format=cl)
    scratch = _workspace(x, (n * (planes * h * w + 2 * co * ho * wo) + 1) // 2, "fbk_fwd")
    CALLS["conv_fwd"] += 3 + (ws[3] is not None)
    check(lib.afan_frozen_bottleneck_fwd(_ptr(x), n, h, w, cin, planes, int(stride), _ptr(ws[0]), _ptr(ws[1]), _ptr(ws[2]), _ptr(ws[3]),
                                         _ptr(ks[0]), _ptr(ks[1]), _ptr(ks[2]), _ptr(ks[3]), _ptr(scratch), _ptr(a1), _ptr(a2),
                                         _ptr(out), _stream(x)), "afan_frozen_bottleneck_fwd")
    return out, a1, a2


class FrozenBlockPlan:
    __slots__ = ("n", "cin", "h", "w", "ho", "wo", "planes", "co", "stride", "fwd_scratch", "bwd_scratch", "wgrad_ws", "w_ptrs", "k_ptrs",
                 "wt_ptrs", "al_ptrs", "gw_ptrs", "n_fwd", "n_wgrad", "has_ds", "keep", "sig")


def frozen_bottleneck_plan(x, planes, stride, ws, ks, wts, als, gws):
    lib = _lib.load()
    p = FrozenBlockPlan()
    p.n, p.cin, p.h, p.w = (int(v) for v in x.shape)
    p.ho, p.wo = (p.h - 1) // stride + 1, (p.w - 1) // stride + 1
    p.planes, p.co, p.stride = int(planes), 4 * int(planes), int(stride)
    p.fwd_scratch = (p.n * (p.planes * p.h * p.w + 2 * p.co * p.ho * p.wo) + 1) // 2
    p.bwd_scratch = (lib.afan_frozen_bottleneck_bwd_scratch(p.n, p.h, p.w, p.cin, p.planes, p.stride) + 1) // 2
    shapes = ((p.n, p.ho, p.wo, p.planes, p.co, 1, 1), (p.n, p.h, p.w, p.planes, p.planes, 3, p.stride), (p.n, p.h, p.w, p.cin, p.planes, 1, 1),
              (p.n, p.h, p.w, p.cin, p.co, 1, p.stride))
    p.wgrad_ws = sum(lib.afan_conv_wgrad_workspace_floats(*sh) for sh, gw in zip(shapes, (gws[2], gws[1], gws[0], gws[3])) if gw is not None)
    p.w_ptrs, p.k_ptrs = tuple(_ptr(t) for t in ws), tuple(_ptr(t) for t in ks)
    p.wt_ptrs, p.al_ptrs, p.gw_ptrs = tuple(_ptr(t) for t in wts), tuple(_ptr(t) for t in als), tuple(_ptr(t) for t in gws)
    p.has_ds = ws[3] is not None
    p.n_fwd, p.n_wgrad = 3 + int(p.has_ds), sum(gw is not None for gw in gws)
    p.keep = (ws, ks, wts, als, gws)
    p.sig = (p.n, p.cin, p.h, p.w, p.planes, p.stride) + tuple(None if t is None else t.data_ptr() for grp in p.keep for t in grp)
    return p
# ... 1242 lines not shown
```

cv_a-fan_amd/resnet_s.py:

```python
import contextlib
import os

import torch
import torch.nn as nn
import torch.nn.functional as F

from . import ops

__all__ = ["ResNet", "ResNet50", "BasicBlock", "Bottleneck", "resnet20", "resnet56", "resnet18", "resnet50", "ARCHS",
           "dgrad_only"]


class _Flags:
    param_grads = True
    weight_epoch = 0
    block_fusion = True
    wgrad_stash = False
    bn_groups = 1
    bn_branch = "main"


@contextlib.contextmanager
def dgrad_only():
    old = _Flags.param_grads
    _Flags.param_grads = False
    try:
        yield
    finally:
        _Flags.param_grads = old


@contextlib.contextmanager
def bn_groups(g):
    old = _Flags.bn_groups
    _Flags.bn_groups = int(g)
    try:
        yield
    finally:
        _Flags.bn_groups = old


def enable_dual_bn(model):
    bns = [m for m in model.modules() if isinstance(m, BatchNorm2d)]
    for b in bns:
        b.enable_dual()
    model._dual_bns = bns
    return model


@contextlib.contextmanager
def bn_branch(model, branch):
    bns = getattr(model, "_dual_bns", None)
    if not bns:
        yield
        return
    old = _Flags.bn_branch
    for b in bns:
        b.select(branch)
    _Flags.bn_branch = branch
    try:
        yield
    finally:
        for b in bns:
            b.select(old)
        _Flags.bn_branch = old


def _bn_fwd_g(raw, b, res, relu, st, G, mom):
    if G == 1 or st.acc is not None:
        return ops.bn_train_forward(raw, b.weight, b.bias, res, relu, b.eps, mom, b.running_mean, b.running_var,
                                    b.num_batches_tracked, st, groups=G)
    c, n = raw.shape[1], raw.shape[0] // G
    y = torch.empty_like(raw)
    stats = torch.empty(G, 4, c, dtype=torch.float32, device=raw.device)
    for g in range(G):
        sl = slice(g * n, (g + 1) * n)
        ops.bn_train_forward(raw[sl], b.weight, b.bias, None if res is None else res[sl], relu, b.eps, mom,
                             b.running_mean, b.running_var, b.num_batches_tracked, st.group(g, c), out=y[sl],
                             stats_out=stats[g])
    return y, stats


def _bn_bwd_g(dy, raw, y, stats, b, relu, want_dres, pg, part, G, dx_out=None):
    gw, gb = (b.weight.grad, b.bias.grad) if pg else (None, None)
    if G == 1 or (part is not None and part.acc is not None):
        return ops.bn_backward(dy, raw, y, stats, b.weight, b.bias, relu, want_dres, gw, gb, pg, partials=part, groups=G,
                               dx_out=dx_out)
    c, n = raw.shape[1], raw.shape[0] // G
    dx = torch.empty_like(raw)
    dres = torch.empty_like(raw) if want_dres else None
    for g in range(G):
        sl = slice(g * n, (g + 1) * n)
        ops.bn_backward(dy[sl], raw[sl], None if y is None else y[sl], stats[g], b.weight, b.bias, relu, want_dres, gw, gb,
                        pg, partials=None if part is None else part.group(g, c), dx_out=dx[sl],
                        dres_out=dres[sl] if want_dres else None)
    return dx, dres


class _CastFn(torch.autograd.Function):

    @staticmethod
    def forward(ctx, x):
        return ops.cast_bf16(x)

    @staticmethod
    def backward(ctx, g):
        return g.float()


def _to_compute(x, dtype):
    if x.dtype == dtype:
        return x
    if x.dtype == torch.float32 and dtype == torch.bfloat16:
        return _CastFn.apply(_dense(x))
    return x.to(dtype)


def _dense(t):
    if t.is_contiguous() or (t.dim() == 4 and t.is_contiguous(memory_format=torch.channels_last)):
        return t
    return t.contiguous()


def _like_layout(t, ref):
    if t.stride() == ref.stride():
        return t
    if ref.dim() == 4 and ops.layout_of(ref) == ops.AFAN_NHWC:
        return t.contiguous(memory_format=torch.channels_last)
    return t.contiguous()


def _sq(v, what):
    if v[0] != v[1]:
        raise ops.AfanLibraryError(f"convolution with a non-square {what} {tuple(v)} is not implemented by libafan_hip")
    return int(v[0])


class _ConvFn(torch.autograd.Function):

    @staticmethod
    def forward(ctx, x, w_master, w_lp, wt_fn, stride, padding, want_wgrad, stats_req=None, dilation=(1, 1), bias=None):
        ctx.stride, ctx.padding, ctx.want_wgrad, ctx.wt_fn = stride, padding, want_wgrad, wt_fn
        ctx.dilation = dilation = tuple(dilation)
        ctx.w_master = w_master
        ctx.own = _own_conv_ok(x, w_lp, stride, padding, dilation) and bias is None
        ctx.has_bias = bias is not None
        if ctx.own:
            ctx.save_for_backward(x, w_lp)
            if stats_req is not None:
                G = _Flags.bn_groups
                if G != 1 and not ops._conv_acc_ok(w_lp.shape[0]):
                    stats_req.append(None)
                    return ops.conv_fwd(x, w_lp, stride[0], dilation=dilation[0])
                y, st = ops.conv_fwd(x, w_lp, stride[0], stats_shift=stats_req[0], want_stats=True,
                                     stats_buf=stats_req[1], dilation=dilation[0], groups=G)
                stats_req.append(st)
                return y
            return ops.conv_fwd(x, w_lp, stride[0], dilation=dilation[0])
        x = _dense(x)
        ctx.save_for_backward(x, w_lp)
        return ops.conv_general_fwd(x, w_lp, None if bias is None else bias.detach().float(), _sq(stride, "stride"),
                                    _sq(padding, "padding"), _sq(dilation, "dilation"))

# ... 618 lines not shown
        return _ConvFn.apply(x, self.weight, self.lp_weight().detach(), self.lp_weight_t, self.stride, self.padding,
                             _Flags.param_grads, None, self.dilation)

    _stats_buf = None
    _bwd_buf = None

    def forward_with_stats(self, x, bn):
        if not (bn.training and self.compute_dtype == torch.bfloat16):
            return self.forward(x), None
        x = _to_compute(x, self.compute_dtype)
        req = [bn.running_mean if bn.track_running_stats else None, self._stats_buf]
        y = _ConvFn.apply(x, self.weight, self.lp_weight().detach(), self.lp_weight_t, self.stride, self.padding,
                          _Flags.param_grads, req, self.dilation)
        st = req[2] if len(req) > 2 else None
        if st is not None:
            self._stats_buf = st.partials
        return y, st


class BatchNorm2d(nn.BatchNorm2d):
    _branch = "main"

    def enable_dual(self):
        if getattr(self, "adv", None) is None:
            aux = nn.BatchNorm2d(self.num_features, eps=self.eps, momentum=self.momentum).to(self.weight.device)
            aux.load_state_dict({k: v.clone() for k, v in nn.BatchNorm2d.state_dict(self).items() if not k.startswith("adv.")})
            self.adv = aux

    def select(self, branch):
        if getattr(self, "adv", None) is None or branch == self._branch:
            return
        a = self.adv
        for k in ("weight", "bias"):
            self._parameters[k], a._parameters[k] = a._parameters[k], self._parameters[k]
        for k in ("running_mean", "running_var", "num_batches_tracked"):
            self._buffers[k], a._buffers[k] = a._buffers[k], self._buffers[k]
        self._branch = branch

    def fused(self, x, residual=None, relu=False, conv_stats=None):
        if self.training:
            mom = self.momentum if self.momentum is not None else 0.1
            G = _Flags.bn_groups
            if G != 1 and (x.shape[0] % G or not x.is_cuda):
                raise ValueError("grouped BatchNorm statistics: the batch must split into equal half-batches on the GPU")
            return _BNTrainFn.apply(x, self.weight, self.bias, residual, relu, self.eps, mom, self.running_mean,
                                    self.running_var, self.num_batches_tracked, _Flags.param_grads, conv_stats, G)
        if torch.is_grad_enabled() and (x.requires_grad or self.weight.requires_grad and _Flags.param_grads):
            if x.requires_grad:
                raise NotImplementedError("eval-mode BatchNorm backward is not on the A-FAN path (the reference "
                                          "runs PGD and the joint step in train mode, main_perturb.py:159)")
        with torch.no_grad():
            invstd = torch.rsqrt(self.running_var + self.eps)
            x = _dense(x)
            return ops.bn_apply(x, self.running_mean, invstd, self.weight, self.bias,
                                None if residual is None else _like_layout(residual, x), relu)

    def forward(self, x):
        return self.fused(x)


class _PadShortcut(nn.Module):

    def __init__(self, planes):
        super().__init__()
        self.pad = planes // 4

    def forward(self, x):
        return F.pad(x[:, :, ::2, ::2], (0, 0, 0, 0, self.pad, self.pad), "constant", 0)


class BasicBlock(nn.Module):
    expansion = 1

    def __init__(self, in_planes, planes, stride=1, option="A"):
        super().__init__()
        self.conv1 = Conv2d(in_planes, planes, kernel_size=3, stride=stride, padding=1, bias=False)
        self.bn1 = BatchNorm2d(planes)
        self.conv2 = Conv2d(planes, planes, kernel_size=3, stride=1, padding=1, bias=False)
        self.bn2 = BatchNorm2d(planes)
        self.shortcut = nn.Sequential()
        self._sc_kind = "identity"
        if stride != 1 or in_planes != planes:
            if option == "A":
                self.shortcut = _PadShortcut(planes)
                self._sc_kind = "pad"
            else:
                self.shortcut = nn.Sequential(
                    Conv2d(in_planes, self.expansion * planes, kernel_size=1, stride=stride, bias=False),
                    BatchNorm2d(self.expansion * planes))
                self._sc_kind = "conv"

    def _chain(self):
        return [(self.conv1, self.bn1), (self.conv2, self.bn2)]

    def forward(self, x):
        x = _to_compute(x, self.conv1.compute_dtype)
        if _Flags.block_fusion and _block_fast_path_ok(self, x):
            return _BlockFn.apply(x, self, _Flags.param_grads, *_block_params(self))
        out, st = self.conv1.forward_with_stats(x, self.bn1)
        out = self.bn1.fused(out, None, True, st)
        out, st = self.conv2.forward_with_stats(out, self.bn2)
        sc = self.shortcut
        if isinstance(sc, nn.Sequential) and len(sc) == 2:
            r, st_sc = sc[0].forward_with_stats(x, sc[1])
            res = sc[1].fused(r, None, False, st_sc)
        else:
            res = sc(x)
        return self.bn2.fused(out, res, True, st)


class Bottleneck(nn.Module):
    expansion = 4

    def __init__(self, in_planes, planes, stride=1, option="B"):
        super().__init__()
        out_planes = planes * 4
        self.conv1 = Conv2d(in_planes, planes, kernel_size=1, stride=1, padding=0, bias=False)
        self.bn1 = BatchNorm2d(planes)
        self.conv2 = Conv2d(planes, planes, kernel_size=3, stride=stride, padding=1, bias=False)
        self.bn2 = BatchNorm2d(planes)
        self.conv3 = Conv2d(planes, out_planes, kernel_size=1, stride=1, padding=0, bias=False)
        self.bn3 = BatchNorm2d(out_planes)
        self.shortcut = nn.Sequential()
        self._sc_kind = "identity"
        if stride != 1 or in_planes != out_planes:
            self.shortcut = nn.Sequential(Conv2d(in_planes, out_planes, kernel_size=1, stride=stride, bias=False),
                                          BatchNorm2d(out_planes))
            self._sc_kind = "conv"

    def _chain(self):
        return [(self.conv1, self.bn1), (self.conv2, self.bn2), (self.conv3, self.bn3)]

    def forward(self, x):
        x = _to_compute(x, self.conv1.compute_dtype)
        if _Flags.block_fusion and _block_fast_path_ok(self, x):
            return _BlockFn.apply(x, self, _Flags.param_grads, *_block_params(self))
        out, st = self.conv1.forward_with_stats(x, self.bn1)
        out = self.bn1.fused(out, None, True, st)
        out, st = self.conv2.forward_with_stats(out, self.bn2)
        out = self.bn2.fused(out, None, True, st)
        out, st = self.conv3.forward_with_stats(out, self.bn3)
        if len(self.shortcut) == 2:
            r, st_sc = self.shortcut[0].forward_with_stats(x, self.shortcut[1])
            res = self.shortcut[1].fused(r, None, False, st_sc)
        else:
            res = x
        return self.bn3.fused(out, res, True, st)


class _HeadFn(torch.autograd.Function):

    @staticmethod
    def forward(ctx, x, weight, bias, want_pgrad):
        logits, pooled = ops.head_forward(x, weight, bias)
        ctx.save_for_backward(x, weight, pooled)
        ctx.bias, ctx.pg = bias, want_pgrad
        return logits

    @staticmethod
    def backward(ctx, g):
        x, weight, pooled = ctx.saved_tensors
        bias = ctx.bias
        want_p = ctx.pg and ctx.needs_input_grad[1]
        dw = db = None
        direct = False
        if want_p:
            direct = _accumulates_in_place(weight) and (bias is None or _accumulates_in_place(bias))
            if direct:
                dw, db = weight.grad, (bias.grad if bias is not None else None)
            else:
                dw = torch.empty_like(weight)
                db = torch.empty_like(bias) if bias is not None else None
        dx = ops.head_backward(g.float().contiguous(), weight, pooled, x, ctx.needs_input_grad[0], dw, db, accumulate=direct)
        if direct:
            dw = db = None
        return dx, dw, db, None


class _CEFn(torch.autograd.Function):

    @staticmethod
    def forward(ctx, logits, target):
        loss, dlogits = ops.cross_entropy(logits, target)
        ctx.save_for_backward(dlogits)
        return loss.reshape(())

    @staticmethod
    def backward(ctx, g):
        (dlogits,) = ctx.saved_tensors
        if g.data_ptr() == ops.one(g.device).data_ptr():
            return dlogits, None
        return dlogits * g, None


_FUSED_CE = os.environ.get("AFAN_FUSED_CE", "1") != "0"


def fused_criterion(criterion, model):
    if not (_FUSED_CE and type(criterion) is nn.CrossEntropyLoss and criterion.weight is None and criterion.ignore_index == -100
            and criterion.reduction == "mean" and getattr(criterion, "label_smoothing", 0.0) == 0.0
            and getattr(model, "compute_dtype", torch.float32) == torch.bfloat16):
        return criterion

    def ce(out, y):
        if (out.is_cuda and out.dtype == torch.float32 and out.dim() == 2 and out.is_contiguous() and y.dtype == torch.int64
                and y.dim() == 1 and 0 < out.numel() <= ops.CE_MAX_ELEMS):
            return _CEFn.apply(out, y)
        return criterion(out, y)
    return ce


_FUSED_HEAD = os.environ.get("AFAN_FUSED_HEAD", "1") != "0"


def _head_ok(x, lin):
    return (_FUSED_HEAD and x.is_cuda and x.dim() == 4 and x.dtype in (torch.float32, torch.bfloat16) and lin.weight.dtype == torch.float32
            and (x.is_contiguous(memory_format=torch.channels_last) and not x.is_contiguous() or x.shape[2] * x.shape[3] == 1)
            and lin.out_features <= 16)


def _head_in(x):
    if x.is_cuda and x.dim() == 4 and x.is_contiguous() and x.shape[2] * x.shape[3] > 1 and x.shape[1] > 1:
        return x.contiguous(memory_format=torch.channels_last)
    return x


class _LinearFn(torch.autograd.Function):

    @staticmethod
    def forward(ctx, x, weight, bias, want_pgrad):
        x = x.contiguous()
        ctx.save_for_backward(x, weight)
        ctx.pg, ctx.bias = want_pgrad, bias
        n, ci = x.shape
        co = weight.shape[0]
        if ci >= 1024 and n <= 1024 and x.dtype == torch.float32 and weight.dtype == torch.float32:
            yt = ops.conv_general_wgrad(x.view(1, n, ci, 1), weight.detach().contiguous().view(1, co, ci, 1), 1)
            y = yt.view(co, n).t()
            return (y + bias.detach()) if bias is not None else y.contiguous()
        y = ops.conv_general_fwd(x.view(n, ci, 1, 1), weight.detach().view(co, ci, 1, 1),
                                 None if bias is None else bias.detach())
        return y.view(n, -1)

    @staticmethod
    def backward(ctx, g):
        x, weight = ctx.saved_tensors
        n, ci = x.shape
        co = weight.shape[0]
        g = g.contiguous().float()
        gx = gw = gb = None
        if ctx.needs_input_grad[0]:
            if co >= 512 and n <= 1024 and weight.dtype == torch.float32 and weight.is_contiguous():
                w_cl = weight.detach().view(1, co, 1, ci).permute(0, 3, 1, 2)
                g_cl = g.t().contiguous().view(1, co, 1, n).permute(0, 3, 1, 2)
                gx = ops.conv_general_wgrad(w_cl, g_cl, 1).reshape(n, ci)
            else:
                gx = ops.conv_general_dgrad(g.view(n, co, 1, 1), weight.detach().view(co, ci, 1, 1), (1, 1)).view(n, ci)
        if ctx.pg and ctx.needs_input_grad[1]:
            direct = _accumulates_in_place(weight)
            gwt = ops.conv_general_wgrad(x.view(n, ci, 1, 1), g.view(n, co, 1, 1), 1,
                                         grad=weight.grad.view(co, ci, 1, 1) if direct else None, accumulate=direct)
            gw = None if direct else gwt.view(co, ci)
            bias = ctx.bias
            if bias is not None:
                if _accumulates_in_place(bias):
                    bias.grad.add_(g.sum(dim=0))
                else:
                    gb = g.sum(dim=0)
        return gx, gw, gb, None


def _linear(x, lin):
    if x.is_cuda and x.dim() == 2 and x.dtype == torch.float32 and lin.weight.dtype == torch.float32:
        return _LinearFn.apply(x, lin.weight, lin.bias, _Flags.param_grads)
    return lin(x)


class _HeadPool(nn.AdaptiveAvgPool2d):

    def forward(self, x):
        return x.float().mean(dim=(2, 3), keepdim=True)


class ResNet(nn.Module):

    def __init__(self, block, num_blocks, num_classes=10, init_weight=1, widths=(16, 32, 64), option="A"):
        super().__init__()
        self.all_layers = 9
        layers = [NormalizeByChannelMeanStd(mean=[0.4914, 0.4822, 0.4465], std=[0.2470, 0.2435, 0.2616]),
                  Conv2d(3, widths[0], kernel_size=3, stride=1, padding=1, bias=False),
                  BatchNorm2d(widths[0]), nn.ReLU()]
        in_planes = widths[0]
        for stage, (planes, nb) in enumerate(zip(widths, num_blocks)):
            for b in range(nb):
                layers.append(block(in_planes, planes, 2 if (stage > 0 and b == 0) else 1, option))
                in_planes = planes * block.expansion
        layers += [_HeadPool((1, 1)), nn.Flatten(), nn.Linear(in_planes, num_classes)]
        self.sequential_model = nn.Sequential(*layers)
        self.w = nn.Parameter(torch.full((self.all_layers,), float(init_weight)), requires_grad=True)
        for m in self.modules():
            if isinstance(m, (nn.Linear, nn.Conv2d)):
                nn.init.kaiming_normal_(m.weight)
        self.compute_dtype = torch.float32
        self.channels_last = False

    def set_channels_last(self, on=True):
        self.channels_last = bool(on)
        for m in self.modules():
            if isinstance(m, NormalizeByChannelMeanStd):
                m.channels_last = self.channels_last
        return self

    @property
    def layer_number(self):
        return len(self.sequential_model)

    def set_compute_dtype(self, dtype):
        if dtype not in (torch.float32, torch.bfloat16):
            raise ValueError("compute dtype must be torch.float32 or torch.bfloat16")
        self.compute_dtype = dtype
        for m in self.modules():
            if isinstance(m, Conv2d):
                m.compute_dtype = dtype
            elif isinstance(m, NormalizeByChannelMeanStd):
                m.out_dtype = dtype
        return self

    def forward(self, x, end_point=34, start_point=0):
        layers = list(self.sequential_model[start_point:end_point])
        if self.channels_last and x.dim() == 4 and x.is_floating_point():
            x = x if x.is_contiguous(memory_format=torch.channels_last) else \
                x.contiguous(memory_format=torch.channels_last)
        i, n = 0, len(layers)
        while i < n:
            L = layers[i]
            if isinstance(L, BatchNorm2d):
                x = _to_compute(x, self.compute_dtype)
                if i + 1 < n and isinstance(layers[i + 1], nn.ReLU):
                    x = L.fused(x, None, True)
                    i += 2
                    continue
                x = L.fused(x)
            elif (isinstance(L, _HeadPool) and i + 2 < n and isinstance(layers[i + 1], nn.Flatten)
                  and isinstance(layers[i + 2], nn.Linear) and _head_ok(_head_in(x), layers[i + 2])):
                lin = layers[i + 2]
                x = _HeadFn.apply(_head_in(x), lin.weight, lin.bias, _Flags.param_grads)
                i += 3
                continue
            elif isinstance(L, nn.Linear):
                x = _linear(x.float(), L)
            else:
                x = L(x)
            i += 1
        return x


class ResNet50(ResNet):

    def __init__(self, num_classes=1000, blocks=(3, 4, 6, 3), init_weight=1):
        nn.Module.__init__(self)
        from .deeplab import MaxPool2d, StemConv
# ... 38 lines not shown
```

cv_a-fan_amd/train_step.py:

```python
import torch
import torch.distributed as dist

from . import ops
from .arena import ArenaSGD, ParamArena
from .attack_algo import PGD, last_norms
from .grid_guard import GuardedTrainer


def warmup_lr(step, optimizer, warm_up_steps=200, max_lr=0.1):
    lr = step * max_lr / (warm_up_steps - 1)
    lr = min(lr, max_lr)
    for p in optimizer.param_groups:
        p["lr"] = lr
    return lr


class GradAllReducer:

    def __init__(self, arena, n_chunks=4, group=None):
        self.arena, self.group = arena, group
        self.world = dist.get_world_size(group) if dist.is_initialized() else 1
        self.chunks = _cut_chunks(arena, n_chunks)
        self.on_cuda = arena.grad.device.type == "cuda"
        self.stream = torch.cuda.Stream(device=arena.grad.device) if self.on_cuda else None
        self._pending = []
        self._hooks = []
        self._need, self._done = [], []
        self.diag = False
        self._diag_ranges, self._diag_wait, self._diag_host = [], None, []
        if self.world > 1:
            bounds = arena.offsets + [arena.numel]
            for ci, (start, end, first_param) in enumerate(self.chunks):
                members = [i for i in range(len(arena.params)) if start <= bounds[i] < end]
                self._need.append(len(members))
                self._done.append(0)
                for i in members:
                    self._hooks.append(arena.params[i].register_post_accumulate_grad_hook(self._make_hook(ci)))

    enabled = False

    def _make_hook(self, ci):
        def hook(_param):
            if not self.enabled:
                return
            self._done[ci] += 1
            if self._done[ci] == self._need[ci]:
                start, end, _ = self.chunks[ci]
                self._launch(start, end)
        return hook

    def begin(self, explicit=False):
        self.enabled = not explicit
        self._done = [0] * len(self.chunks)
        self._covered = []
        self._diag_ranges, self._diag_wait, self._diag_host = [], None, []
        ops.exchange_in_flight(False)

    def launch_params(self, p_lo, p_hi):
        if p_hi <= p_lo:
            return
        bounds = self.arena.offsets + [self.arena.numel]
        start, end = bounds[p_lo], bounds[p_hi]
        self._covered.append((start, end))
        self._launch(start, end)

    def _launch(self, start, end):
        buf = self.arena.grad[start:end]
        ops.exchange_in_flight(True)
        if self.on_cuda:
            ev = torch.cuda.Event(enable_timing=self.diag)
            ev.record(torch.cuda.current_stream(buf.device))
            with torch.cuda.stream(self.stream):
                self.stream.wait_event(ev)
                if self.diag:
                    e0, e1 = torch.cuda.Event(enable_timing=True), torch.cuda.Event(enable_timing=True)
                    e0.record(self.stream)
                w = dist.all_reduce(buf, op=dist.ReduceOp.SUM, group=self.group, async_op=True)
                if self.diag:
                    if self.world > 1 and dist.get_backend(self.group) != "nccl":
                        w.wait()
                    e1.record(self.stream)
                    self._diag_ranges.append((start, end, ev, e0, e1))
        else:
            w = dist.all_reduce(buf, op=dist.ReduceOp.SUM, group=self.group, async_op=True)
        self._pending.append(w)

    _covered = ()

    def finish(self):
        self.enabled = False
        if self._covered:
            pos = 0
            for start, end in sorted(self._covered):
                if start > pos:
                    self._launch(pos, start)
                pos = max(pos, end)
            if pos < self.arena.numel:
                self._launch(pos, self.arena.numel)
            self._covered = []
        else:
            for ci, (start, end, _) in enumerate(self.chunks):
                if self._done[ci] < self._need[ci]:
                    self._launch(start, end)
        cur = torch.cuda.current_stream(self.arena.grad.device) if self.on_cuda else None
        if self.diag and self.on_cuda:
            wa, wb = torch.cuda.Event(enable_timing=True), torch.cuda.Event(enable_timing=True)
            wa.record(cur)
        for w in self._pending:
            w.wait()
        self._pending.clear()
        if self.on_cuda:
            cur.wait_stream(self.stream)
            if self.diag:
                wb.record(cur)
                self._diag_wait = (wa, wb)
        ops.exchange_in_flight(False)

    def note_host_gap(self, seconds):
        if self.diag:
            self._diag_host.append(seconds)

    def last_diag(self):
        if not (self.diag and self.on_cuda and self._diag_wait):
            return None
        rs = [{"bytes": (end - start) * 4, "queued_ms": round(ev.elapsed_time(e0), 3), "allreduce_ms": round(e0.elapsed_time(e1), 3)}
              for start, end, ev, e0, e1 in self._diag_ranges]
        return {"ranges": rs, "exposed_allreduce_ms": round(self._diag_wait[0].elapsed_time(self._diag_wait[1]), 3),
                "host_gap_us": [round(h * 1e6, 1) for h in self._diag_host]}


class NullReducer:
    world = 1
    diag = False
    stream = None

    def __init__(self, arena):
        self.arena = arena
        self.announced = []
        self.fused_while_in_flight = 0
        self._mark = None

    def begin(self, explicit=False):
        self.announced, self._mark = [], None
        ops.exchange_in_flight(False)

    def launch_params(self, p_lo, p_hi):
        if p_hi <= p_lo:
            return
        self.announced.append((p_lo, p_hi))
        if self._mark is None:
            self._mark = ops.CALLS["conv_bn_fused"]
        ops.exchange_in_flight(True)

    def finish(self):
        if self._mark is not None:
            self.fused_while_in_flight += ops.CALLS["conv_bn_fused"] - self._mark
        ops.exchange_in_flight(False)

    def note_host_gap(self, seconds):
        pass

    def last_diag(self):
        return None


def _cut_chunks(arena, n_chunks):
    bounds = arena.offsets + [arena.numel]
    target = arena.numel / max(n_chunks, 1)
    cuts, end = [], arena.numel
    for i in range(len(arena.offsets) - 1, -1, -1):
        if end - bounds[i] >= target or i == 0:
            cuts.append((bounds[i], end, i))
            end = bounds[i]
    return cuts


def _out_shape(mod, c, h, w):
    import torch.nn as nn
    if isinstance(mod, nn.Conv2d):
        st = mod.stride[0]
        return mod.out_channels, (h + 2 * mod.padding[0] - mod.kernel_size[0]) // st + 1, (w + 2 * mod.padding[1] - mod.kernel_size[1]) // st + 1
    if isinstance(mod, nn.MaxPool2d):
        k, st, p = mod.kernel_size, mod.stride, mod.padding
        return c, (h + 2 * p - k) // st + 1, (w + 2 * p - k) // st + 1
    if hasattr(mod, "_chain"):
        for conv, _ in mod._chain():
            st = conv.stride[0]
            h, w = (h + st - 1) // st, (w + st - 1) // st
            c = conv.out_channels
        return c, h, w
    return c, h, w


class AfanTrainer(GuardedTrainer):

    def __init__(self, model, criterion, *, steps=5, gamma=0.5, eps=2.0, perturb_idx=13, layer_number=None,
                 randinit=False, clip=False, lr=0.1, momentum=0.9, weight_decay=5e-4, allreduce_chunks=4,
                 group=None, use_graph=True, graph_warmup=3, batch_final=True,
                 share_head=True, fold_clean=None, segmented=None, dual_bn=False, emulate_dp=False):
        self.model, self.criterion = model, criterion
        self.dual_bn = bool(dual_bn)
        if self.dual_bn:
            from . import resnet_s
            resnet_s.enable_dual_bn(model)
            fold_clean, batch_final = False, False
        self.steps, self.gamma, self.eps = steps, gamma, eps
        self.perturb_idx = perturb_idx
        self.layer_number = layer_number if layer_number is not None else model.layer_number
        self.randinit, self.clip = randinit, clip
        self.arena = ParamArena(model)
        self.optimizer = ArenaSGD(self.arena, lr, momentum, weight_decay)
        self.group = group
        self.world = dist.get_world_size(group) if dist.is_initialized() else 1
        self.reducer = GradAllReducer(self.arena, allreduce_chunks, group) if self.world > 1 else None
        if self.world > 1:
            self.optimizer.grad_scale = 1.0 / self.world
            self.sync_replicas()
        elif emulate_dp:
            self.reducer = NullReducer(self.arena)
        self._guard_init(model, self.arena.param.device)
        import os
        self.ddp_overlap = self.reducer is not None and os.environ.get("AFAN_DDP_OVERLAP", "1") != "0"
        self.segmented = bool(segmented)
        self._pieces = None
        self.batch_final = bool(batch_final)
        self._groupable_key, self._groupable = None, False
        self.share_head = bool(share_head)
        self.fold_clean = fold_clean if fold_clean is None else bool(fold_clean)
        self._fold_auto = {}
        self.use_graph = bool(use_graph) and not randinit
        self.graph_warmup = graph_warmup
        self._graph = None
        self._graph_failed = None
        self._graph_unsafe = None
        self._eager_steps = 0
        self._static_in = None
        self._static_out = None
        self._shape_key = None
        self._stream = None

    def sync_replicas(self, src=0):
        if not dist.is_initialized() or self.world <= 1:
            return
        a = self.arena
        for t in (a.param, a.momentum_buf):
            dist.broadcast(t, src=src, group=self.group)
        for b in self.model.buffers():
            dist.broadcast(b, src=src, group=self.group)
        a.refresh_shadow()

    FOLD_MIN_ELEMS = 0

    def _fold_ok(self, inp):
        if self.fold_clean is False or not (self._share_head(inp) and self.steps >= 1 and not self.randinit):
            return False
        if self.fold_clean is None:
            key = tuple(inp.shape)
            if self._fold_auto.get(key) is None:
                self._fold_auto[key] = self._feature_elems(inp) >= self.FOLD_MIN_ELEMS
            return self._fold_auto[key]
        return True

    def _feature_elems(self, inp):
        m = self.model
        c, h, w = inp.shape[1], inp.shape[2], inp.shape[3]
        for mod in m.sequential_model[:self.perturb_idx]:
            c, h, w = _out_shape(mod, c, h, w)
        return inp.shape[0] * c * h * w

    def _forward_backward_folded(self, inp, target, overlap_allreduce):
        from . import ops, resnet_s
        m, idx, ln = self.model, self.perturb_idx, self.layer_number
        ops.acc_reset(inp.device)
        self.optimizer.zero_grad()
        crit = resnet_s.fused_criterion(self.criterion, m)
        half = ops.half(inp.device)
        with ops.bn_running_updates(2):
            fm_clean = m(inp, end_point=idx, start_point=0)
        xin = fm_clean.detach().requires_grad_(True)
        with ops.record_bn_updates() as clean_bn:
            output_clean = m(xin, end_point=ln, start_point=idx)
        loss_clean = crit(output_clean, target)
        with resnet_s.stash_wgrad():
            torch.autograd.backward(loss_clean, grad_tensors=half)
        g0 = xin.grad
        feature_map = fm_clean.detach()
        feature_map = feature_map.float() if feature_map.dtype != torch.float32 else feature_map
        feature_map_adv = PGD(feature_map, self.criterion, y=target, model=m, steps=self.steps,
                              gamma=(self.gamma / 255), start_idx=idx, layer_number=ln, eps=(self.eps / 255),
                              randinit=False, clip=self.clip, with_norms=True, grad0=g0)
        l2, linf = last_norms()
        adv_in = getattr(feature_map_adv, "_afan_shadow", None)
        if adv_in is None:
            adv_in = feature_map_adv.detach()
        output_adv = m(adv_in, end_point=ln, start_point=idx)
        loss_adv = crit(output_adv, target)
        torch.autograd.backward(loss_adv, grad_tensors=half)
        resnet_s.flush_wgrad(m)
        clean_bn.replay()
        if overlap_allreduce:
            self.reducer.begin()
        fm_clean.backward(g0)
        with torch.no_grad():
            loss = (loss_adv + loss_clean) / 2
            prec1 = (output_clean.argmax(dim=1) == target).float().sum() * (100.0 / target.shape[0])
        return {"loss": loss.detach(), "loss_adv": loss_adv.detach(), "loss_clean": loss_clean.detach(),
                "prec1": prec1, "l2": l2, "linf": linf, "x_adv": feature_map_adv.detach(),
                "feature_map": feature_map, "out_clean": output_clean.detach()}

    def _tail_segments(self):
        m, idx, ln = self.model, self.perturb_idx, self.layer_number
        cuts = [idx]
        for i in range(idx + 1, ln):
            mod = m.sequential_model[i]
            if getattr(mod, "_sc_kind", "identity") != "identity":
                cuts.append(i)
        cuts.append(ln)
        return [(cuts[k], cuts[k + 1]) for k in range(len(cuts) - 1)]

    def _param_range(self, a, b):
        pre = tuple(f"sequential_model.{i}." for i in range(a, b))
        idxs = [i for i, n in enumerate(self.arena.names) if n.startswith(pre)]
        return (idxs[0], idxs[-1] + 1) if idxs else (0, 0)

    def _phases_folded(self, inp, target, out):
        from . import ops, resnet_s
        m, idx, ln = self.model, self.perturb_idx, self.layer_number
        segs = self._tail_segments()
        ops.acc_reset(inp.device)
        self.optimizer.zero_grad()
        crit = resnet_s.fused_criterion(self.criterion, m)
        half = ops.half(inp.device)

        def run_segments(x0):
            ins, outs, h = [x0], [], x0
            for k, (a, b) in enumerate(segs):
                o = m(h, end_point=b, start_point=a)
                outs.append(o)
                if k + 1 < len(segs):
                    h = o.detach().requires_grad_(True)
                    ins.append(h)
            return ins, outs

        with ops.bn_running_updates(2):
            fm_clean = m(inp, end_point=idx, start_point=0)
        xin = fm_clean.detach().requires_grad_(True)
        with ops.record_bn_updates() as clean_bn:
            c_ins, c_outs = run_segments(xin)
        loss_clean = crit(c_outs[-1], target)
        with resnet_s.stash_wgrad():
            torch.autograd.backward(loss_clean, grad_tensors=half)
            for k in range(len(segs) - 2, -1, -1):
                c_outs[k].backward(c_ins[k + 1].grad)
        g0 = xin.grad
        feature_map = fm_clean.detach()
        feature_map = feature_map.float() if feature_map.dtype != torch.float32 else feature_map
        feature_map_adv = PGD(feature_map, self.criterion, y=target, model=m, steps=self.steps,
                              gamma=(self.gamma / 255), start_idx=idx, layer_number=ln, eps=(self.eps / 255),
                              randinit=False, clip=self.clip, with_norms=True, grad0=g0)
        l2, linf = last_norms()
        adv_in = getattr(feature_map_adv, "_afan_shadow", None)
        if adv_in is None:
            adv_in = feature_map_adv.detach()
        a_ins, a_outs = run_segments(adv_in)
        loss_adv = crit(a_outs[-1], target)
        torch.autograd.backward(loss_adv, grad_tensors=half)
        resnet_s.flush_wgrad(m.sequential_model[segs[-1][0]:segs[-1][1]])
        yield self._param_range(*segs[-1])
        with ops.grid_bn(self.reducer is None):
            for k in range(len(segs) - 2, -1, -1):
                a_outs[k].backward(a_ins[k + 1].grad)
                resnet_s.flush_wgrad(m.sequential_model[segs[k][0]:segs[k][1]])
                if k == 0:
                    clean_bn.replay()
                yield self._param_range(*segs[k])
            if len(segs) == 1:
                clean_bn.replay()
            fm_clean.backward(g0)
        with torch.no_grad():
            loss = (loss_adv + loss_clean) / 2
            prec1 = (c_outs[-1].argmax(dim=1) == target).float().sum() * (100.0 / target.shape[0])
        out.update({"loss": loss.detach(), "loss_adv": loss_adv.detach(), "loss_clean": loss_clean.detach(),
                    "prec1": prec1, "l2": l2, "linf": linf, "x_adv": feature_map_adv.detach(),
                    "feature_map": feature_map, "out_clean": c_outs[-1].detach()})
        yield self._param_range(0, idx)

    def _ddp_phases_ok(self, inp):
        want = self.segmented or (self.ddp_overlap and self.reducer is not None)
        return bool(want and self._fold_ok(inp) and hasattr(self.model, "sequential_model"))

    def _forward_backward(self, inp, target, overlap_allreduce):
        if self._fold_ok(inp):
            return self._forward_backward_folded(inp, target, overlap_allreduce)
        m, idx, ln = self.model, self.perturb_idx, self.layer_number
        if inp.is_cuda:
            from . import ops
            ops.acc_reset(inp.device)
        fm_clean = None
        if self._share_head(inp):
            from . import ops
            with ops.bn_running_updates(2):
                fm_clean = m(inp, end_point=idx, start_point=0)
            feature_map = fm_clean.detach()
        else:
            with torch.no_grad():
                feature_map = m(inp, end_point=idx, start_point=0)
        feature_map = feature_map.float() if feature_map.dtype != torch.float32 else feature_map
        from . import resnet_s as _rsb
        with _rsb.bn_branch(m, "adv"):
            feature_map_adv = PGD(feature_map, self.criterion, y=target, model=m, steps=self.steps,
                                  gamma=(self.gamma / 255), start_idx=idx, layer_number=ln, eps=(self.eps / 255),
                                  randinit=self.randinit, clip=self.clip, with_norms=True)
        l2, linf = last_norms()
        adv_in = getattr(feature_map_adv, "_afan_shadow", None)
        if adv_in is None:
            adv_in = feature_map_adv.detach()
        if self.batch_final and self._tail_groupable(adv_in):
            from . import resnet_s
            if fm_clean is None:
                fm_clean = m(inp, end_point=idx, start_point=0)
            both = torch.cat([adv_in, fm_clean.to(adv_in.dtype)], dim=0)
            with resnet_s.bn_groups(2):
                out_both = m(both, end_point=ln, start_point=idx)
            nb = adv_in.shape[0]
            output_adv, output_clean = out_both[:nb], out_both[nb:]
        else:
            with _rsb.bn_branch(m, "adv"):
                output_adv = m(adv_in, end_point=ln, start_point=idx)
            output_clean = (m(fm_clean, end_point=ln, start_point=idx) if fm_clean is not None
                            else m(inp, end_point=ln, start_point=0))
        from . import resnet_s as _rs
        crit = _rs.fused_criterion(self.criterion, m)
        loss_adv = crit(output_adv.contiguous() if output_adv.dim() == 2 else output_adv, target)
        loss_clean = crit(output_clean.contiguous() if output_clean.dim() == 2 else output_clean, target)
        loss = (loss_adv + loss_clean) / 2
        self.optimizer.zero_grad()
        if overlap_allreduce:
            self.reducer.begin()
        from . import resnet_s
        if loss.is_cuda and loss.dtype == torch.float32 and loss.dim() == 0:
            from . import ops as _ops
            loss.backward(gradient=_ops.one(loss.device))
        else:
            loss.backward()
        with torch.no_grad():
            prec1 = (output_clean.argmax(dim=1) == target).float().sum() * (100.0 / target.shape[0])
        return {"loss": loss.detach(), "loss_adv": loss_adv.detach(), "loss_clean": loss_clean.detach(),
                "prec1": prec1, "l2": l2, "linf": linf, "x_adv": feature_map_adv.detach(),
                "feature_map": feature_map, "out_clean": output_clean.detach()}

    def _share_head(self, inp):
        m = self.model
        return bool(self.share_head and inp.is_cuda and self.perturb_idx > 0 and getattr(m, "channels_last", False)
                    and hasattr(m, "sequential_model") and m.training)

    def _tail_groupable(self, fea):
        from . import ops as _ops
        key = (tuple(fea.shape), fea.dtype, fea.is_contiguous(memory_format=torch.channels_last), _ops.BN_ACC)
        if self._groupable_key == key:
            return self._groupable
        from . import resnet_s
        from . import ops
        ok = (fea.is_cuda and fea.dim() == 4 and fea.dtype == torch.bfloat16 and key[2] and resnet_s._Flags.block_fusion
              and ops.BN_ACC)
        n, _, h, w = fea.shape if fea.dim() == 4 else (0, 0, 0, 0)
        if ok:
            for mod in self.model.sequential_model[self.perturb_idx:self.layer_number]:
                if isinstance(mod, (resnet_s.BasicBlock, resnet_s.Bottleneck)):
                    probe = torch.empty((2, mod._chain()[0][0].in_channels, 2, 2), dtype=torch.bfloat16,
                                        device=fea.device).contiguous(memory_format=torch.channels_last)
                    if not (mod.training and resnet_s._block_fast_path_ok(mod, probe)):
                        ok = False
                        break
                    for c, _ in mod._chain():
                        if (n * h * w) % 128 or (c.stride[0] == 2 and ((h | w) & 1)):
                            ok = False
                        h, w = (h + c.stride[0] - 1) // c.stride[0], (w + c.stride[0] - 1) // c.stride[0]
                        if (n * h * w) % 128:
                            ok = False
                    if not ok:
                        break
                elif any(isinstance(q, torch.nn.modules.batchnorm._BatchNorm) for q in mod.modules()):
                    ok = False
                    break
        self._groupable_key, self._groupable = key, bool(ok)
        return self._groupable

    def _graph_safe(self):
        if self._graph_unsafe is None:
            from . import resnet_s
            self._graph_unsafe = resnet_s.vendor_convs(self.model) if hasattr(self.model, "sequential_model") else []
            if self._graph_unsafe:
                self.use_graph = False
        return not self._graph_unsafe

    def _step_eager(self, inp, target):
        self.optimizer._sync_lr()
        if self._ddp_phases_ok(inp):
            out = {}
            if self.reducer is not None:
                self.reducer.begin(explicit=True)
            for rng in self._phases_folded(inp, target, out):
                if self.reducer is not None:
                    self.reducer.launch_params(*rng)
            if self.reducer is not None:
                self.reducer.finish()
            self._pre_sgd()
            self.optimizer.step()
            return out
        out = self._forward_backward(inp, target, overlap_allreduce=self.reducer is not None)
        if self.reducer is not None:
            self.reducer.finish()
        self._pre_sgd()
        self.optimizer.step()
        return out

    def _pre_sgd(self):
        if self._guard is not None and self.world > 1:
            self._guard.sync_ranks(self.group)

    def _drop_graphs(self):
        self._graph = self._pieces = self._static_in = self._static_out = self._shape_key = None
        self._graph_failed = None

    def _capture_pieces(self, inp, target):
        dev = inp.device
        self._stream = torch.cuda.Stream(device=dev)
        self._static_in = (inp.clone(), target.clone())
        self._stream.wait_stream(torch.cuda.current_stream(dev))
        torch.cuda.synchronize(dev)
        out, pieces, pool, fused = {}, [], None, []
        gen = self._phases_folded(self._static_in[0], self._static_in[1], out)
        try:
            for _ in range(len(self._tail_segments()) + 1):
                n0 = ops.CALLS["conv_bn_fused"]
                g = torch.cuda.CUDAGraph()
                with ops.no_gc_during_capture(), torch.cuda.graph(g, pool=pool, stream=self._stream, capture_error_mode="thread_local"):
                    rng = next(gen)
                fused.append(ops.CALLS["conv_bn_fused"] - n0)
                pieces.append((g, rng))
                pool = pieces[0][0].pool()
                if self.reducer is not None:
                    ops.exchange_in_flight(True)
        finally:
            ops.exchange_in_flight(False)
        gen.close()
        self._pieces_fused = fused
        self._pieces, self._static_out = pieces, out
        self._graph = pieces[0][0]
        self._shape_key = (tuple(inp.shape), inp.dtype, tuple(target.shape))

    def _capture(self, inp, target):
        if self._ddp_phases_ok(inp):
            return self._capture_pieces(inp, target)
        dev = inp.device
        self._stream = torch.cuda.Stream(device=dev)
        self._static_in = (inp.clone(), target.clone())
        self._stream.wait_stream(torch.cuda.current_stream(dev))
        g = torch.cuda.CUDAGraph()
        with ops.no_gc_during_capture(), torch.cuda.graph(g, stream=self._stream, capture_error_mode="thread_local"):
            out = self._forward_backward(self._static_in[0], self._static_in[1], overlap_allreduce=False)
            if self.world == 1:
                self.optimizer.step()
        self._graph, self._static_out = g, out
        self._shape_key = (tuple(inp.shape), inp.dtype, tuple(target.shape))
# ... 48 lines not shown
```

include/afan_hip.h:

```cpp
#ifndef AFAN_HIP_H
#define AFAN_HIP_H

#include <stdint.h>

#ifdef __cplusplus
extern "C" {
#endif

typedef void* afan_stream_t;

enum { AFAN_F32 = 0, AFAN_BF16 = 1 };

enum { AFAN_NCHW = 0, AFAN_NHWC = 1 };

enum {
    AFAN_OK = 0,
    AFAN_EDTYPE = -1,
    AFAN_EALIGN = -2,
    AFAN_ESHAPE = -3,
    AFAN_ENULL = -4,
    AFAN_ELAYOUT = -5
};

int afan_version(void);
// ... 137 lines not shown
                                    const void* bn_y, double* bn_acc, float* dweight, float* dbias, int accumulate, void* barrier,
                                    afan_stream_t stream);
int64_t afan_conv_dgrad_tiles(int64_t n, int64_t hi, int64_t wi, int64_t ci, int64_t co, int k, int stride);

int64_t afan_conv_wgrad_workspace_floats(int64_t n, int64_t hi, int64_t wi, int64_t ci, int64_t co, int k, int stride);
int afan_conv_wgrad_nhwc_bf16(const void* x, const void* dy, float* grad, int64_t n, int64_t hi, int64_t wi,
                              int64_t ci, int64_t co, int k, int stride, int dilation, float* workspace, int accumulate,
                              afan_stream_t stream);
int afan_conv_wgrad2_nhwc_bf16(const void* x, const void* dy, int64_t n, const void* x2, const void* dy2, int64_t n2,
                               float* grad, int64_t hi, int64_t wi, int64_t ci, int64_t co, int k, int stride, int dilation,
                               float* workspace, int accumulate, afan_stream_t stream);

int afan_conv_wgrad_plan(int64_t n, int64_t hi, int64_t wi, int64_t ci, int64_t co, int k, int stride);
int afan_conv_wgrad_multi_nhwc_bf16(int nb, const void* const* x, const void* const* dy, float* const* grad, const int64_t* n,
                                    const int64_t* hi, const int64_t* wi, const int64_t* ci, const int64_t* co, const int* k,
                                    const int* stride, const int* dilation, float* workspace, int accumulate,
                                    afan_stream_t stream);

int afan_conv_fwd(const void* x, const void* w, const float* bias, void* y, int dtype, int layout, int w_layout, int64_t n,
                  int64_t hi, int64_t wi, int64_t ci, int64_t co, int k, int stride, int pad, int dilation, afan_stream_t stream);
int afan_conv_dgrad(const void* dy, const void* w, void* dx, int dtype, int layout, int w_layout, int64_t n, int64_t hi,
                    int64_t wi, int64_t ci, int64_t co, int k, int stride, int pad, int dilation, afan_stream_t stream);
int64_t afan_conv_wgrad_f32_workspace_floats(int64_t n, int64_t hi, int64_t wi, int64_t ci, int64_t co, int k, int stride,
                                             int pad, int dilation);
int afan_conv_wgrad(const void* x, const void* dy, float* grad, int dtype, int layout, int w_layout, int64_t n, int64_t hi,
                    int64_t wi, int64_t ci, int64_t co, int k, int stride, int pad, int dilation, float* workspace,
                    int accumulate, afan_stream_t stream);

int afan_conv_stem7_supported(int64_t ci, int64_t co, int k, int stride);
int afan_conv_stem7_fwd_nhwc_bf16(const void* x, const void* w, void* y, int64_t n, int64_t hi, int64_t wi,
                                  afan_stream_t stream);
int afan_conv_stem7_im2col_k(void);
int afan_conv_stem7_im2col(const void* x, void* cols, int64_t n, int64_t hi, int64_t wi, afan_stream_t stream);
int afan_conv_stem7_col2im(const void* dcols, void* dx, int64_t n, int64_t hi, int64_t wi, afan_stream_t stream);
int64_t afan_conv_stem7_wgrad_workspace_floats(int64_t n, int64_t hi, int64_t wi);
int afan_conv_stem7_wgrad_nhwc_bf16(const void* x, const void* dy, float* grad, int64_t n, int64_t hi, int64_t wi,
                                    float* workspace, int accumulate, afan_stream_t stream);

int afan_upsample_bilinear_fwd(const void* x, void* y, int dtype, int layout, int64_t n, int64_t c, int64_t hi, int64_t wi,
                               int64_t ho, int64_t wo, afan_stream_t stream);
int afan_upsample_bilinear_bwd(const void* dy, void* dx, int dtype, int layout, int64_t n, int64_t c, int64_t hi, int64_t wi,
                               int64_t ho, int64_t wo, afan_stream_t stream);
int afan_upsample_bilinear_fwd_slice(const void* x, void* y, int dtype, int64_t n, int64_t c, int64_t hi, int64_t wi, int64_t ho,
                                     int64_t wo, int64_t ld, afan_stream_t stream);
int64_t afan_upsample_bilinear_bwd_workspace_floats(int64_t n, int64_t c, int64_t wi, int64_t ho);
int afan_upsample_bilinear_bwd_slice(const void* dy, void* dx, int dtype, int64_t n, int64_t c, int64_t hi, int64_t wi, int64_t ho,
                                     int64_t wo, int64_t ld, float* ws, afan_stream_t stream);
int64_t afan_ce2d_workspace_floats(int64_t pixels);
int afan_ce2d(const float* logits, const int64_t* target, int layout, int64_t n, int64_t c, int64_t hw, int64_t ignore_index,
              float grad_scale, float* workspace, float* loss, float* dlogits, afan_stream_t stream);
int64_t afan_ce2d_upsampled_workspace_floats(int64_t n, int64_t c, int64_t h, int64_t w, int64_t ho, int64_t wo);
int afan_ce2d_upsampled(const float* logits, const int64_t* target, int64_t n, int64_t c, int64_t h, int64_t w, int64_t ho,
                        int64_t wo, int64_t ignore_index, float grad_scale, float* workspace, float* loss, float* dlogits,
                        afan_stream_t stream);
int afan_maxpool3x3s2_fwd(const void* x, void* y, int dtype, int layout, int64_t n, int64_t c, int64_t hi, int64_t wi,
                          afan_stream_t stream);
int afan_maxpool3x3s2_bwd(const void* dy, const void* x, void* dx, int dtype, int layout, int64_t n, int64_t c, int64_t hi,
                          int64_t wi, afan_stream_t stream);
int afan_maxpool2d_fwd(const void* x, void* y, uint8_t* idx, int dtype, int layout, int64_t n, int64_t c, int64_t hi, int64_t wi,
                       int k, int stride, int pad, afan_stream_t stream);
int afan_maxpool2d_bwd(const void* dy, const void* x, const uint8_t* idx, void* dx, int dtype, int layout, int64_t n, int64_t c,
                       int64_t hi, int64_t wi, int k, int stride, int pad, afan_stream_t stream);
int afan_affine_relu_bwd(const void* dy, const void* y, const float* alpha, void* dx, void* dres, int dtype, int layout,
                         int64_t n, int64_t c, int64_t hw, int relu, afan_stream_t stream);
int afan_affine_coefs(const float* mean, const float* invstd, const float* weight, const float* bias, int64_t c,
                      float* coefs, afan_stream_t stream);
int afan_affine_apply(const void* x, const void* residual, void* y, int dtype, int64_t n, int64_t c, int64_t hw,
                      const float* coefs, int relu, afan_stream_t stream);

int afan_frozen_bottleneck_fwd(const void* x, int64_t n, int64_t h, int64_t w, int64_t cin, int64_t planes, int stride,
                               const void* w1, const void* w2, const void* w3, const void* wd, const float* k1, const float* k2,
                               const float* k3, const float* kd, void* scratch, void* a1, void* a2, void* out,
                               afan_stream_t stream);
int64_t afan_frozen_bottleneck_bwd_scratch(int64_t n, int64_t h, int64_t w, int64_t cin, int64_t planes, int stride);
int afan_frozen_bottleneck_bwd(const void* g, const void* x, const void* a1, const void* a2, const void* out, int64_t n,
                               int64_t h, int64_t w, int64_t cin, int64_t planes, int stride, const void* wt1, const void* wt2,
                               const void* wt3, const void* wtd, const float* al1, const float* al2, const float* al3,
                               const float* ald, float* gw1, float* gw2, float* gw3, float* gwd, float* wgrad_ws, void* scratch,
                               void* dx, afan_stream_t stream);
int afan_frozen_bottleneck_bwd_chain(const void* g, void* pre_d3, void* pre_dres, const void* x, const void* a1, const void* a2,
                                     const void* out, int64_t n, int64_t h, int64_t w, int64_t cin, int64_t planes, int stride,
                                     const void* wt1, const void* wt2, const void* wt3, const void* wtd, const float* al1, const float* al2,
                                     const float* al3, const float* ald, float* gw1, float* gw2, float* gw3, float* gwd, float* wgrad_ws,
                                     void* scratch, void* dx, const float* prev_al3, void* prev_d3, void* prev_dres, afan_stream_t stream);
int afan_avgpool_fwd(const void* x, void* y, int dtype, int layout, int64_t n, int64_t c, int64_t hw, int pooled_f32,
                     afan_stream_t stream);
int afan_avgpool_bwd(const void* dy, void* dx, int dtype, int layout, int64_t n, int64_t c, int64_t hw, int pooled_f32,
                     afan_stream_t stream);
int afan_linear_small_max_rows(void);
int afan_linear_small_fwd(const float* x, const float* w, float* y, int64_t n, int64_t ci, int64_t co, afan_stream_t stream);
int afan_linear_small_bwd(const float* dy, const float* x, const float* w, float* dx, float* dw, int64_t n, int64_t ci,
                          int64_t co, int accumulate, afan_stream_t stream);
int afan_pointwise_max_co(void);
int afan_pointwise_fwd(const void* x, int x_dtype, const float* w, const float* b, float* y, int64_t m, int64_t ci,
                       int64_t co, afan_stream_t stream);
int afan_pointwise_bwd_dx(const float* dy, const float* w, void* dx, int dx_dtype, int64_t m, int64_t ci, int64_t co,
                          afan_stream_t stream);
int64_t afan_pointwise_workspace_floats(int64_t m, int64_t ci, int64_t co);
int afan_pointwise_bwd_dw(const float* dy, const void* x, int x_dtype, float* dw, float* db, int64_t m, int64_t ci,
                          int64_t co, float* workspace, int accumulate, afan_stream_t stream);
int afan_dropout(const void* x, void* y, int dtype, int64_t n, float p, const uint8_t* mask, uint64_t* state, uint64_t* used,
                 int advance, afan_stream_t stream);

int64_t afan_nms_workspace_bytes(int64_t n);
int afan_nms(const float* boxes, const int64_t* order, int64_t n, float threshold, int inclusive, void* workspace,
             int64_t* keep_out, int64_t* count_out, afan_stream_t stream);
int afan_nms_top(const float* boxes, const int64_t* order, int64_t n, float threshold, int inclusive, void* workspace,
                 int64_t* keep_out, int64_t* count_out, int64_t max_keep, afan_stream_t stream);

int afan_box_decode_clip(const float* src, const float* t, float* out, int64_t n, float right, float bottom, afan_stream_t stream);
int afan_box_assign(const float* boxes, const float* gt, int64_t B, int64_t N, int64_t G, int mode, float lo, float hi,
                    const int64_t* gt_classes, int64_t* labels, int64_t* assign, void* workspace, afan_stream_t stream);
int afan_sample_lists(const int64_t* labels, int64_t M, int64_t* fg, int64_t* bg, int64_t* counts, afan_stream_t stream);
int afan_sample_gather(const int64_t* fg, const int64_t* bg, const int64_t* pos, int64_t S, const float* boxes, const float* gt,
                       const int64_t* assign, const int64_t* labels, int64_t N, int64_t G, int64_t* sel, float* out_boxes,
                       int64_t* out_labels, float* out_deltas, int64_t* out_batch, afan_stream_t stream);
int afan_det_loss_fwd(const float* logits, const float* deltas, const int64_t* rows, const int64_t* gt_labels, const float* gt_deltas,
                      const int64_t* batch, int64_t S, int64_t B, int64_t C, int64_t K, float beta, const float* norm, float* ce, float* sl1,
                      float* save, afan_stream_t stream);
int afan_sum_scalars_f32(const float* a, const float* b, const float* c, const float* d, float* out, afan_stream_t stream);
int64_t afan_linear_pair_workspace_floats(int op, int64_t M, int64_t n1, int64_t n2, int64_t K);
int afan_linear_pair_fwd_f32(const float* x, const float* w1, const float* b1, const float* w2, const float* b2, float* y1, float* y2, int64_t M,
                             int64_t n1, int64_t n2, int64_t K, float* ws, afan_stream_t stream);
int afan_linear_pair_dgrad_f32(const float* g1, const float* g2, const float* w1, const float* w2, float* gx, int64_t M, int64_t n1, int64_t n2,
                               int64_t K, afan_stream_t stream);
int afan_linear_pair_wgrad_f32(const float* g1, const float* g2, const float* x, float* gw1, float* gb1, float* gw2, float* gb2, int accumulate,
                               int64_t M, int64_t n1, int64_t n2, int64_t K, float* ws, afan_stream_t stream);
int afan_proposal_rows(const float* cand, int64_t n_cand, const int64_t* keep, int64_t n_keep, const int64_t* count, int64_t P,
                       float* rows, int64_t* kept, afan_stream_t stream);
int afan_labels_limit(int64_t* labels, int64_t B, int64_t N, const int64_t* kept, int64_t n_kept, afan_stream_t stream);
int afan_det_loss_bwd(const float* g_ce, const float* g_sl1, const float* save, const int64_t* rows, const int64_t* gt_labels,
                      const int64_t* batch, int64_t S, int64_t B, int64_t C, int64_t K, int64_t R, float* d_logits, float* d_deltas,
                      afan_stream_t stream);
int afan_roi_align_fwd(const void* x, const float* rois, void* y, int dtype, int layout, int64_t num_rois, int64_t c, int64_t h,
                       int64_t w, int pooled_h, int pooled_w, float spatial_scale, int sampling_ratio, afan_stream_t stream);
int afan_roi_align_bwd(const void* dy, const float* rois, float* dx, int dtype, int layout, int64_t num_rois, int64_t n, int64_t c,
                       int64_t h, int64_t w, int pooled_h, int pooled_w, float spatial_scale, int sampling_ratio,
                       afan_stream_t stream);
int64_t afan_roi_align_bwd_workspace_bytes(int64_t num_rois, int64_t h, int64_t w);
int afan_roi_align_bwd_ws(const void* dy, const float* rois, float* dx, int dtype, int layout, int64_t num_rois, int64_t n, int64_t c,
                          int64_t h, int64_t w, int pooled_h, int pooled_w, float spatial_scale, int sampling_ratio, void* workspace,
                          afan_stream_t stream);

int afan_head_max_classes(void);
int afan_head_forward(const void* x, int dtype, int64_t n, int64_t c, int64_t hw, const float* weight, const float* bias,
                      int64_t k, float* pooled, float* logits, afan_stream_t stream);
int afan_head_backward(const float* dlogits, const float* weight, const float* pooled, int64_t n, int64_t c, int64_t hw,
                       int64_t k, void* dx, int dx_dtype, float* dweight, float* dbias, int accumulate,
                       afan_stream_t stream);

int afan_cross_entropy(const float* logits, const int64_t* target, int64_t n, int64_t k, float* loss, float* dlogits,
                       afan_stream_t stream);

int afan_transpose_weights(const void* src_arena, void* dst_arena, const int64_t* desc_dev, int n_desc,
                           int64_t total_tiles, afan_stream_t stream);

int afan_sgd_step(float* param, const float* grad, float* momentum_buf, uint16_t* shadow_bf16,
                  int64_t n, const float* lr_dev, float momentum, float weight_decay,
                  float grad_scale, int first_step, afan_stream_t stream);

int afan_sgd_step_guarded(float* param, const float* grad, float* momentum_buf, uint16_t* shadow_bf16,
                          int64_t n, const float* lr_dev, float momentum, float weight_decay,
                          float grad_scale, int first_step, const void* guard, afan_stream_t stream);
int afan_guarded_copy(void* dst, const void* src, int64_t bytes, const void* guard, void* counter, afan_stream_t stream);
int afan_occupy_cus(int workgroups, int lds_bytes, int microseconds, afan_stream_t stream);

int afan_cast_bf16(const float* src, uint16_t* dst, int64_t n, afan_stream_t stream);
int afan_pgd_init(const void* x, int dtype, float* x32, float* x_adv, uint16_t* shadow, int64_t n, afan_stream_t stream);
int afan_normalize_nchw(const float* x, void* y, int out_dtype, int out_layout, int64_t n, int64_t c, int64_t hw,
                        const float* mean, const float* std, afan_stream_t stream);

int afan_profile_enable(int on);
int afan_profile_collect(char* names_out, int64_t* launches, double* total_ms, double* total_bytes,
                         double* total_flops, int max_kernels);
int afan_profile_event_overhead(int n, float* us_out, afan_stream_t stream);

int afan_conv_trace(int on);
int afan_conv_trace_read(int64_t* problems, char* names, int max_records);

#ifdef __cplusplus
}
#endif
#endif
```

Baseline: 33270 images/sec.

## Fuse classifier head with cross-entropy and fold first PGD step into init

Adds a single head_ce kernel that does average pooling, the linear head, softmax cross-entropy, dlogits, the input gradient, and a last-block reduction of loss, prec1 and the joint loss, using an atomic ticket. The clean, PGD and adversarial head passes now run through it via a head_loss context. It also adds pgd_init_step, which merges the bf16-to-fp32 init with the first PGD step that uses grad0, and drops the separate float cast and the argmax/mean observables. The aim is fewer kernel launches and fewer memory passes over small tensors in a launch-bound step, at the cost of ticket-based cross-block coordination and extra bookkeeping for when the fused record applies.

```diff
diff --git a/cv_a-fan_amd/_lib.py b/cv_a-fan_amd/_lib.py
--- a/cv_a-fan_amd/_lib.py
+++ b/cv_a-fan_amd/_lib.py
@@ -29,6 +29,7 @@
     "afan_head_forward": (_i, [_p, _i, _l, _l, _l, _p, _p, _l, _p, _p, _p]),
     "afan_head_backward": (_i, [_p, _p, _p, _l, _l, _l, _l, _p, _i, _p, _p, _i, _p]),
     "afan_cross_entropy": (_i, [_p, _p, _l, _l, _p, _p, _p]),
+    "afan_head_ce": (_i, [_p, _i, _l, _l, _l, _p, _p, _l, _p, _p, _p, _p, _p, _p, _p, _p, _p, _p, _p, _p, _p]),
     "afan_mix_w_workspace_floats": (_l, []),
     "afan_mix_w": (_i, [_p, _p, _p, _p, _i, _l, _p]),
     "afan_mix_w_backward": (_i, [_p, _i, _p, _p, _l, _p, _p, _i, _p]),
@@ -144,6 +145,7 @@
     "afan_occupy_cus": (_i, [_i, _i, _i, _p]),
     "afan_cast_bf16": (_i, [_p, _p, _l, _p]),
     "afan_pgd_init": (_i, [_p, _i, _p, _p, _p, _l, _p]),
+    "afan_pgd_init_step": (_i, [_p, _i, _p, _i, _p, _p, _p, _l, _f, _f, _i, _p]),
     "afan_normalize_nchw": (_i, [_p, _p, _i, _i, _l, _l, _l, _p, _p, _p]),
     "afan_profile_enable": (_i, [_i]),
     "afan_profile_collect": (_i, [C.c_char_p, C.POINTER(_l), C.POINTER(C.c_double), C.POINTER(C.c_double),
diff --git a/cv_a-fan_amd/attack_algo.py b/cv_a-fan_amd/attack_algo.py
--- a/cv_a-fan_amd/attack_algo.py
+++ b/cv_a-fan_amd/attack_algo.py
@@ -1,7 +1,7 @@
 import torch
 
 from . import ops
-from .resnet_s import _dense, _like_layout, dgrad_only, fused_criterion
+from .resnet_s import _dense, _like_layout, dgrad_only, fused_criterion, head_loss
 
 __all__ = ["PGD", "tensor_clamp", "linfball_proj", "mix_feature", "get_sample_points", "last_norms"]
 
@@ -32,7 +32,13 @@
     lp = getattr(model, "compute_dtype", torch.float32) == torch.bfloat16
     if grad0 is not None and (randinit or steps < 1):
         raise ValueError("grad0 is the gradient at x: not with randinit, and only when there is a first step")
-    x, x_adv, shadow = ops.pgd_init(_dense(x.detach()), want_shadow=lp and grad0 is None and not randinit)
+    first = 0
+    if grad0 is not None and ops.HEAD_CE and not (with_norms and steps == 1):
+        x = _dense(x.detach())
+        x, x_adv, shadow = ops.pgd_init_step(x, _like_layout(grad0.detach(), x), gamma, eps, clip, want_shadow=lp)
+        first = 1
+    else:
+        x, x_adv, shadow = ops.pgd_init(_dense(x.detach()), want_shadow=lp and grad0 is None and not randinit)
     if lp and shadow is None:
         shadow = torch.empty_like(x, dtype=torch.bfloat16)
     if randinit:
@@ -40,13 +46,15 @@
         ops.axpy_noise_(x_adv, u, eps, shadow)
     l2 = linf = None
     loss_fn = fused_criterion(loss_fn, model)
-    for t in range(steps):
+    one = ops.one(x.device) if getattr(loss_fn, "_afan_fused", False) else None
+    for t in range(first, steps):
         if t == 0 and grad0 is not None:
             grad = grad0.detach()
         else:
             xin = (shadow if lp else x_adv).detach().requires_grad_(True)
             with dgrad_only():
-                out = model(xin, end_point=layer_number, start_point=start_idx)
+                with head_loss(y, one):
+                    out = model(xin, end_point=layer_number, start_point=start_idx)
                 loss = loss_fn(out, y)
                 root = ops.one(loss.device) if (loss.dim() == 0 and loss.dtype == torch.float32) else None
                 grad = torch.autograd.grad(loss, xin, grad_outputs=root, only_inputs=True)[0]
@@ -60,6 +68,7 @@
             l2, linf = ops.perturb_norms(x_adv, x)
         _last["l2"], _last["linf"] = l2, linf
     x_adv.requires_grad_(True)
+    x_adv._afan_x32 = x
     if lp:
         x_adv._afan_shadow = shadow
     return x_adv
diff --git a/cv_a-fan_amd/csrc/afan_head.hip b/cv_a-fan_amd/csrc/afan_head.hip
--- a/cv_a-fan_amd/csrc/afan_head.hip
+++ b/cv_a-fan_amd/csrc/afan_head.hip
@@ -191,11 +191,194 @@
     }
 }
 
+typedef __attribute__((address_space(1))) unsigned long long gu64_t;
+typedef __attribute__((address_space(1))) unsigned gu32_t;
+
+struct HeadCeArgs {
+    const void* x; const float* W; const float* bias; const int64_t* target; const float* root;
+    float* pooled; float* logits; float* dlogits; void* dx;
+    unsigned long long* rows;
+    unsigned* ticket;
+    float* loss;
+    float* prec1;
+    const float* loss_other;
+    float* loss_joint;
+    int N, C, HW, K;
+};
+
+template <typename T, bool VEC>
+__global__ __launch_bounds__(BLOCK) void head_ce_kernel(const HeadCeArgs a) {
+    __shared__ float grp[VEC ? BLOCK * 8 : 1];
+    __shared__ float red[BLOCK / AFAN_WAVE][MAXK];
+    __shared__ float lg[MAXK];
+    __shared__ float dl[MAXK];
+    __shared__ unsigned s_last;
+    const int C = a.C, HW = a.HW, K = a.K, N = a.N;
+    const int b = blockIdx.x;
+    const float* __restrict__ W = a.W;
+    const float inv = 1.0f / (float)HW;
+    float part[MAXK];
+#pragma unroll
+    for (int k = 0; k < MAXK; ++k) part[k] = 0.f;
+    const int P = C >> 3, G = VEC ? BLOCK / P : 1;
+    const int pc = VEC ? threadIdx.x % P : 0, pg = VEC ? threadIdx.x / P : 0;
+    if constexpr (VEC) {
+        const uint16_t* xb = (const uint16_t*)a.x + (int64_t)b * HW * C + pc * 8;
+        float s[8];
+#pragma unroll
+        for (int j = 0; j < 8; ++j) s[j] = 0.f;
+        for (int p = pg; p < HW; p += G) {
+            const u16x8 v = *reinterpret_cast<const u16x8*>(xb + (int64_t)p * C);
+#pragma unroll
+            for (int j = 0; j < 8; ++j) s[j] += bf2f(v[j]);
+        }
+#pragma unroll
+        for (int j = 0; j < 8; ++j) grp[pg * C + pc * 8 + j] = s[j];
+        __syncthreads();
+        for (int c = threadIdx.x; c < C; c += BLOCK) {
+            float t = 0.f;
+            for (int g = 0; g < G; ++g) t += grp[g * C + c];
+            const float m = t * inv;
+            a.pooled[(int64_t)b * C + c] = m;
+#pragma unroll
+            for (int k = 0; k < MAXK; ++k)
+                if (k < K) part[k] = fmaf(m, W[(int64_t)k * C + c], part[k]);
+        }
+    } else {
+        const T* xb = (const T*)a.x + (int64_t)b * HW * C;
+        for (int c = threadIdx.x; c < C; c += BLOCK) {
+            float s = 0.f;
+            for (int p = 0; p < HW; ++p) s += Elt<T>::ld(xb + (int64_t)p * C + c);
+            const float m = s * inv;
+            a.pooled[(int64_t)b * C + c] = m;
+#pragma unroll
+            for (int k = 0; k < MAXK; ++k)
+                if (k < K) part[k] = fmaf(m, W[(int64_t)k * C + c], part[k]);
+        }
+    }
+#pragma unroll
+    for (int k = 0; k < MAXK; ++k) {
+        if (k < K) {
+            const float v = wave_sum(part[k]);
+            if ((threadIdx.x & 63) == 0) red[threadIdx.x >> 6][k] = v;
+        }
+    }
+    __syncthreads();
+    if (threadIdx.x < K) {
+        float t = a.bias ? a.bias[threadIdx.x] : 0.f;
+        for (int w = 0; w < BLOCK / AFAN_WAVE; ++w) t += red[w][threadIdx.x];
+        a.logits[(int64_t)b * K + threadIdx.x] = t;
+        lg[threadIdx.x] = t;
+    }
+    __syncthreads();
+    if (threadIdx.x < K) {
+        const float invn = 1.0f / (float)N;
+        float m = lg[0];
+        for (int k = 1; k < K; ++k) m = fmaxf(m, lg[k]);
+        float s = 0.f;
+        for (int k = 0; k < K; ++k) s += expf(lg[k] - m);
+        const float lse = m + logf(s);
+        const int64_t t64 = a.target[b];
+        const bool bad = t64 < 0 || t64 >= K;
+        const int t = bad ? 0 : (int)t64;
+        const int k = threadIdx.x;
+        float d = bad ? NAN : (expf(lg[k] - lse) - (k == t ? 1.f : 0.f)) * invn;
+        d = d * a.root[0];
+        a.dlogits[(int64_t)b * K + k] = d;
+        dl[k] = d;
+        if (k == 0) {
+            const float rl = bad ? NAN : lse - lg[t];
+            int best = 0;
+            for (int j = 1; j < K; ++j) {
+                const float v = lg[j], w = lg[best];
+                if (v > w || (v != v && w == w)) best = j;
+            }
+            const unsigned long long g = (unsigned long long)__builtin_bit_cast(unsigned, rl) |
+                                         ((unsigned long long)((int64_t)best == t64 ? 1u : 0u) << 32);
+            __hip_atomic_store((gu64_t*)(a.rows + b), g, __ATOMIC_RELAXED, __HIP_MEMORY_SCOPE_AGENT);
+            asm volatile("s_waitcnt vmcnt(0)" ::: "memory");
+            const unsigned tk = __hip_atomic_fetch_add((gu32_t*)a.ticket, 1u, __ATOMIC_RELAXED, __HIP_MEMORY_SCOPE_AGENT);
+            s_last = (tk == (unsigned)(N - 1)) ? 1u : 0u;
+        }
+    }
+    __syncthreads();
+    if (a.dx) {
+        if constexpr (VEC) {
+            for (int c = threadIdx.x; c < C; c += BLOCK) {
+                float g = 0.f;
+                for (int k = 0; k < K; ++k) g = fmaf(dl[k], W[(int64_t)k * C + c], g);
+                g *= inv;
+                grp[c] = g;
+            }
+            __syncthreads();
+            u16x8 o;
+#pragma unroll
+            for (int j = 0; j < 8; ++j) o[j] = f2bf(grp[pc * 8 + j]);
+            uint16_t* xb = (uint16_t*)a.dx + (int64_t)b * HW * C + pc * 8;
+            for (int p = pg; p < HW; p += G) *reinterpret_cast<u16x8*>(xb + (int64_t)p * C) = o;
+        } else {
+            T* xb = (T*)a.dx + (int64_t)b * HW * C;
+            for (int c = threadIdx.x; c < C; c += BLOCK) {
+                float g = 0.f;
+                for (int k = 0; k < K; ++k) g = fmaf(dl[k], W[(int64_t)k * C + c], g);
+                g *= inv;
+                for (int p = 0; p < HW; ++p) Elt<T>::st(xb + (int64_t)p * C + c, g);
+            }
+        }
+    }
+    if (!s_last) return;
+    __shared__ float lred[BLOCK / AFAN_WAVE];
+    __shared__ unsigned hred[BLOCK / AFAN_WAVE];
+    const float invn = 1.0f / (float)N;
+    float local = 0.f;
+    unsigned hits = 0;
+    for (int r = threadIdx.x; r < N; r += BLOCK) {
+        const unsigned long long g = __hip_atomic_load((gu64_t*)(a.rows + r), __ATOMIC_RELAXED, __HIP_MEMORY_SCOPE_AGENT);
+        local += __builtin_bit_cast(float, (unsigned)g);
+        hits += (unsigned)(g >> 32);
+    }
+    const float w = wave_sum(local);
+#pragma unroll
+    for (int o = 32; o > 0; o >>= 1) hits += __shfl_xor(hits, o, 64);
+    if ((threadIdx.x & 63) == 0) { lred[threadIdx.x >> 6] = w; hred[threadIdx.x >> 6] = hits; }
+    __syncthreads();
+    if (threadIdx.x == 0) {
+        float s = 0.f;
+        unsigned h = 0;
+        for (int i = 0; i < BLOCK / AFAN_WAVE; ++i) { s += lred[i]; h += hred[i]; }
+        const float l = s * invn;
+        a.loss[0] = l;
+        if (a.prec1) a.prec1[0] = (float)h * (float)(100.0 / (double)N);
+        if (a.loss_joint) a.loss_joint[0] = (l + a.loss_other[0]) * 0.5f;
+        __hip_atomic_store((gu32_t*)a.ticket, 0u, __ATOMIC_RELAXED, __HIP_MEMORY_SCOPE_AGENT);
+    }
+}
+
 }
 
 extern "C" {
 
 int afan_head_max_classes(void) { return MAXK; }
+
+int afan_head_ce(const void* x, int dtype, int64_t n, int64_t c, int64_t hw, const float* weight, const float* bias, int64_t k,
+                 const int64_t* target, const float* root, float* pooled, float* logits, float* dlogits, void* dx, void* rows,
+                 void* ticket, float* loss, float* prec1, const float* loss_other, float* loss_joint, afan_stream_t stream) {
+    if (dtype != AFAN_F32 && dtype != AFAN_BF16) return AFAN_EDTYPE;
+    if (n <= 0 || c <= 0 || hw <= 0 || k <= 0 || k > MAXK || n * k > (1 << 16) || c % 8 != 0 || n * hw * c > 0x7FFFFFFF) return AFAN_ESHAPE;
+    if (dtype == AFAN_BF16 && !(c / 8 <= BLOCK && BLOCK % (c / 8) == 0 && aligned(x, 16) && (!dx || aligned(dx, 16)))) return AFAN_ESHAPE;
+    if (!x || !weight || !target || !root || !pooled || !logits || !dlogits || !rows || !ticket || !loss) return AFAN_ENULL;
+    if ((loss_joint != nullptr) != (loss_other != nullptr)) return AFAN_ENULL;
+    if (!aligned(rows, 8) || !aligned(ticket, 4)) return AFAN_EALIGN;
+    hipStream_t st = (hipStream_t)stream;
+    const double eb = dtype == AFAN_F32 ? 4 : 2;
+    AFAN_PROF("head_ce_kernel", (double)n * hw * c * eb * (dx ? 2 : 1), st);
+    HeadCeArgs a{x, weight, bias, target, root, pooled, logits, dlogits, dx, (unsigned long long*)rows, (unsigned*)ticket, loss, prec1,
+                 loss_other, loss_joint, (int)n, (int)c, (int)hw, (int)k};
+    if (dtype == AFAN_F32) head_ce_kernel<float, false><<<(unsigned)n, BLOCK, 0, st>>>(a);
+    else head_ce_kernel<uint16_t, true><<<(unsigned)n, BLOCK, 0, st>>>(a);
+    AFAN_LAUNCH_CHECK();
+    return AFAN_OK;
+}
 
 int afan_head_forward(const void* x, int dtype, int64_t n, int64_t c, int64_t hw, const float* weight, const float* bias,
                       int64_t k, float* pooled, float* logits, afan_stream_t stream) {
diff --git a/cv_a-fan_amd/csrc/afan_pgd.hip b/cv_a-fan_amd/csrc/afan_pgd.hip
--- a/cv_a-fan_amd/csrc/afan_pgd.hip
+++ b/cv_a-fan_amd/csrc/afan_pgd.hip
@@ -287,6 +287,72 @@
         x_adv[i] = v;
         if (shadow) shadow[i] = f2bf(v);
     }
+}
+
+template <typename S, typename G, bool CLIP>
+__global__ __launch_bounds__(BLOCK) void pgd_init_step_kernel(const S* __restrict__ x, const G* __restrict__ grad,
+                                                              float* __restrict__ x32, float* __restrict__ x_adv,
+                                                              uint16_t* __restrict__ shadow, int64_t n, float gamma, float eps, int vec) {
+    const int64_t tid = (int64_t)blockIdx.x * BLOCK + threadIdx.x;
+    const int64_t nthreads = (int64_t)gridDim.x * BLOCK;
+    int64_t done = 0;
+    if (vec) {
+        const int64_t nvec = n >> 3;
+        for (int64_t v = tid; v < nvec; v += nthreads) {
+            const int64_t i = v << 3;
+            float o[8], g[8];
+            if constexpr (sizeof(S) == 4) {
+                float a[4], b[4];
+                Elt<float>::ldv((const float*)x + i, a);
+                Elt<float>::ldv((const float*)x + i + 4, b);
+#pragma unroll
+                for (int e = 0; e < 4; ++e) { o[e] = a[e]; o[4 + e] = b[e]; }
+            } else {
+                Elt<uint16_t>::ldv((const uint16_t*)x + i, o);
+            }
+            if constexpr (sizeof(G) == 4) {
+                float a[4], b[4];
+                Elt<float>::ldv((const float*)grad + i, a);
+                Elt<float>::ldv((const float*)grad + i + 4, b);
+#pragma unroll
+                for (int e = 0; e < 4; ++e) { g[e] = a[e]; g[4 + e] = b[e]; }
+            } else {
+                Elt<uint16_t>::ldv((const uint16_t*)grad + i, g);
+            }
+            if (x32) {
+                const float lo[4] = {o[0], o[1], o[2], o[3]}, hi[4] = {o[4], o[5], o[6], o[7]};
+                Elt<float>::stv(x32 + i, lo);
+                Elt<float>::stv(x32 + i + 4, hi);
+            }
+            float t[8];
+#pragma unroll
+            for (int e = 0; e < 8; ++e) t[e] = step_one<CLIP>(o[e], g[e], o[e], gamma, eps);
+            const float lo[4] = {t[0], t[1], t[2], t[3]}, hi[4] = {t[4], t[5], t[6], t[7]};
+            Elt<float>::stv(x_adv + i, lo);
+            Elt<float>::stv(x_adv + i + 4, hi);
+            if (shadow) Elt<uint16_t>::stv(shadow + i, t);
+        }
+        done = nvec << 3;
+    }
+    for (int64_t i = done + tid; i < n; i += nthreads) {
+        const float v = Elt<S>::ld(x + i);
+        if (x32) x32[i] = v;
+        const float t = step_one<CLIP>(v, Elt<G>::ld(grad + i), v, gamma, eps);
+        x_adv[i] = t;
+        if (shadow) shadow[i] = f2bf(t);
+    }
+}
+
+template <typename S, typename G>
+int launch_init_step(const void* x, const void* grad, float* x32, float* x_adv, uint16_t* shadow, int64_t n, float gamma, float eps,
+                     int clip, hipStream_t st) {
+    const int vec = aligned(x, 16) && aligned(grad, 16) && aligned(x_adv, 16) && (!x32 || aligned(x32, 16)) && (!shadow || aligned(shadow, 16));
+    const int grid = grid_for(vec ? (n + 7) / 8 : n, BLOCK);
+    AFAN_PROF("pgd_init_step_kernel", n * (double)(sizeof(S) + sizeof(G) + 4.0 + (x32 ? 4 : 0) + (shadow ? 2 : 0)), st);
+    if (clip) pgd_init_step_kernel<S, G, true><<<grid, BLOCK, 0, st>>>((const S*)x, (const G*)grad, x32, x_adv, shadow, n, gamma, eps, vec);
+    else pgd_init_step_kernel<S, G, false><<<grid, BLOCK, 0, st>>>((const S*)x, (const G*)grad, x32, x_adv, shadow, n, gamma, eps, vec);
+    AFAN_LAUNCH_CHECK();
+    return AFAN_OK;
 }
 
 template <typename G, bool CLIP, bool SHADOW>
@@ -465,4 +531,22 @@
     return AFAN_OK;
 }
 
-}
+int afan_pgd_init_step(const void* x, int dtype, const void* grad, int grad_dtype, float* x32, float* x_adv, uint16_t* shadow,
+                       int64_t n, float gamma, float eps, int clip, afan_stream_t stream) {
+    if ((dtype != AFAN_F32 && dtype != AFAN_BF16) || (grad_dtype != AFAN_F32 && grad_dtype != AFAN_BF16)) return AFAN_EDTYPE;
+    if (n < 0) return AFAN_ESHAPE;
+    if (n == 0) return AFAN_OK;
+    if (!x || !grad || !x_adv || (dtype == AFAN_BF16 && !x32)) return AFAN_ENULL;
+    if (!aligned(x, dtype == AFAN_F32 ? 4 : 2) || !aligned(grad, grad_dtype == AFAN_F32 ? 4 : 2) || !aligned(x_adv, 4) ||
+        (x32 && !aligned(x32, 4)) || (shadow && !aligned(shadow, 2)))
+        return AFAN_EALIGN;
+    hipStream_t st = (hipStream_t)stream;
+    if (dtype == AFAN_F32) {
+        if (grad_dtype == AFAN_F32) return launch_init_step<float, float>(x, grad, x32, x_adv, shadow, n, gamma, eps, clip, st);
+        return launch_init_step<float, uint16_t>(x, grad, x32, x_adv, shadow, n, gamma, eps, clip, st);
+    }
+    if (grad_dtype == AFAN_F32) return launch_init_step<uint16_t, float>(x, grad, x32, x_adv, shadow, n, gamma, eps, clip, st);
+    return launch_init_step<uint16_t, uint16_t>(x, grad, x32, x_adv, shadow, n, gamma, eps, clip, st);
+}
+
+}
diff --git a/cv_a-fan_amd/learnable.py b/cv_a-fan_amd/learnable.py
--- a/cv_a-fan_amd/learnable.py
+++ b/cv_a-fan_amd/learnable.py
@@ -126,11 +126,12 @@
         for num in self.idx_list:
             with torch.no_grad():
                 fea = m(inp, end_point=num, start_point=0)
-            fea = fea.float() if fea.dtype != torch.float32 else fea
-            clean.append(fea)
+            if not ops.HEAD_CE:
+                fea = fea.float() if fea.dtype != torch.float32 else fea
             adv.append(PGD(fea, self.criterion, y=target, model=m, steps=self.steps, gamma=(self.gamma / 255),
                            start_idx=num, layer_number=ln, eps=(self.eps / 255), randinit=self.randinit,
                            clip=self.clip))
+            clean.append(adv[-1]._afan_x32)
         dtype = getattr(m, "compute_dtype", torch.float32)
         outs, l2s, linfs = [], [], []
         for i, num in enumerate(self.idx_list):
diff --git a/cv_a-fan_amd/ops.py b/cv_a-fan_amd/ops.py
--- a/cv_a-fan_amd/ops.py
+++ b/cv_a-fan_amd/ops.py
@@ -320,6 +320,21 @@
     shadow = torch.empty_like(x, dtype=torch.bfloat16) if want_shadow else None
     check(lib.afan_pgd_init(_ptr(x), _DT[x.dtype], None if x32 is x else _ptr(x32), _ptr(x_adv),
                             None if shadow is None else _ptr(shadow), x.numel(), _stream(x)), "afan_pgd_init")
+    return x32, x_adv, shadow
+
+
+def pgd_init_step(x, grad, gamma, eps=0.0, clip=False, want_shadow=False):
+    lib = _lib.load()
+    _need(x, "x"), _need(grad, "grad")
+    if x.dtype not in _DT or grad.dtype not in _DT or grad.numel() != x.numel():
+        raise TypeError("x and grad must be fp32 or bf16 with the same number of elements")
+    _same_layout(x, grad)
+    x32 = x if x.dtype == torch.float32 else torch.empty_like(x, dtype=torch.float32)
+    x_adv = torch.empty_like(x, dtype=torch.float32)
+    shadow = torch.empty_like(x, dtype=torch.bfloat16) if want_shadow else None
+    check(lib.afan_pgd_init_step(_ptr(x), _DT[x.dtype], _ptr(grad), _DT[grad.dtype], None if x32 is x else _ptr(x32), _ptr(x_adv),
+                                 _ptr(shadow), x.numel(), float(gamma), float(eps), int(bool(clip)), _stream(x)),
+          "afan_pgd_init_step")
     return x32, x_adv, shadow
 
 
@@ -430,6 +445,46 @@
                                  _DT[x_like.dtype], _ptr(dweight), _ptr(dbias), int(bool(accumulate)), _stream(x_like)),
           "afan_head_backward")
     return dx
+
+
+HEAD_CE = os.environ.get("AFAN_HEAD_CE", "1") != "0"
+_head_ce_ws = {}
+
+
+def _head_ce_scratch(ref, n):
+    key = (ref.device.index, _raw_stream(ref.device.index))
+    ws = _head_ce_ws.get(key)
+    if ws is None or ws.numel() < 2 + n:
+        ws = _head_ce_ws[key] = torch.zeros(2 + max(int(n), 1024), dtype=torch.int64, device=ref.device)
+    return ws
+
+
+def head_ce(x, weight, bias, target, root, want_dx=True, want_prec1=False, joint_with=None):
+    lib = _lib.load()
+    _need(x, "x"), _need(weight, "weight", torch.float32), _need(root, "root", torch.float32)
+    if x.dim() != 4 or not (layout_of(x) == AFAN_NHWC or x.shape[2] * x.shape[3] == 1) or x.dtype not in _DT:
+        raise ValueError("head_ce: x must be a channels-last fp32/bf16 feature map")
+    n, c, hw = _nchw(x)
+    k = weight.shape[0]
+    if not (target.is_cuda and target.dtype == torch.int64 and target.dim() == 1 and target.shape[0] == n and target.is_contiguous()
+            and root.numel() == 1 and weight.is_contiguous()):
+        raise TypeError("head_ce: target [N] int64 contiguous on the GPU, root one fp32 element")
+    dev = x.device
+    pooled = torch.empty(n, c, dtype=torch.float32, device=dev)
+    logits = torch.empty(n, k, dtype=torch.float32, device=dev)
+    dlogits = torch.empty(n, k, dtype=torch.float32, device=dev)
+    dx = torch.empty_like(x) if want_dx else None
+    small = torch.empty(3, dtype=torch.float32, device=dev)
+    ws = _head_ce_scratch(x, n)
+    rc = lib.afan_head_ce(_ptr(x), _DT[x.dtype], n, c, hw, _ptr(weight), _ptr(bias), k, _ptr(target), _ptr(root), _ptr(pooled),
+                          _ptr(logits), _ptr(dlogits), _ptr(dx), _ptr(ws[2:]), _ptr(ws), _ptr(small[0:1]),
+                          _ptr(small[1:2]) if want_prec1 else None, _ptr(joint_with), _ptr(small[2:3]) if joint_with is not None else None,
+                          _stream(x))
+    if rc == -3:
+        return None
+    check(rc, "afan_head_ce")
+    return {"logits": logits, "pooled": pooled, "loss": small[0:1], "dlogits": dlogits, "dx": dx,
+            "prec1": small[1] if want_prec1 else None, "loss_joint": small[2] if joint_with is not None else None}
 
 
 def bn_stats(x, eps=1e-5, momentum=0.1, running_mean=None, running_var=None, num_batches=None):
diff --git a/cv_a-fan_amd/resnet_s.py b/cv_a-fan_amd/resnet_s.py
--- a/cv_a-fan_amd/resnet_s.py
+++ b/cv_a-fan_amd/resnet_s.py
@@ -8,7 +8,7 @@
 from . import ops
 
 __all__ = ["ResNet", "ResNet50", "BasicBlock", "Bottleneck", "resnet20", "resnet56", "resnet18", "resnet50", "ARCHS",
-           "dgrad_only"]
+           "dgrad_only", "head_loss"]
 
 
 class _Flags:
@@ -933,7 +933,21 @@
 
     @staticmethod
     def forward(ctx, x, weight, bias, want_pgrad):
-        logits, pooled = ops.head_forward(x, weight, bias)
+        ctx.rec = None
+        hl = _HeadLoss.active
+        rec = None
+        if hl is not None and ops.HEAD_CE and _head_loss_ok(x, weight, hl):
+            target, root, want_prec1, joint = hl
+            rec = ops.head_ce(x, weight, None if bias is None else bias.detach(), target, root, want_dx=ctx.needs_input_grad[0],
+                              want_prec1=want_prec1, joint_with=joint)
+        if rec is not None:
+            logits, pooled = rec.pop("logits"), rec.pop("pooled")
+            rec["target"], rec["root_ptr"] = hl[0], hl[1].data_ptr()
+            rec["mark"] = (rec["dlogits"].data_ptr(), rec["dlogits"]._version)
+            rec["logits_mark"] = (logits.data_ptr(), logits._version)
+            ctx.rec = logits._afan_ce = rec
+        else:
+            logits, pooled = ops.head_forward(x, weight, bias)
         ctx.save_for_backward(x, weight, pooled)
         ctx.bias, ctx.pg = bias, want_pgrad
         return logits
@@ -952,26 +966,67 @@
             else:
                 dw = torch.empty_like(weight)
                 db = torch.empty_like(bias) if bias is not None else None
-        dx = ops.head_backward(g.float().contiguous(), weight, pooled, x, ctx.needs_input_grad[0], dw, db, accumulate=direct)
+        rec, ctx.rec = ctx.rec, None
+        if (rec is not None and g.dtype == torch.float32 and (g.data_ptr(), g._version) == rec["mark"] and rec.get("taken")
+                and g.shape == rec["dlogits"].shape and g.is_contiguous()):
+            dx = rec["dx"] if ctx.needs_input_grad[0] else None
+            if dw is not None:
+                ops.head_backward(g, weight, pooled, x, False, dw, db, accumulate=direct)
+        else:
+            dx = ops.head_backward(g.float().contiguous(), weight, pooled, x, ctx.needs_input_grad[0], dw, db, accumulate=direct)
         if direct:
             dw = db = None
         return dx, dw, db, None
 
 
+class _HeadLoss:
+    active = None
+
+
+@contextlib.contextmanager
+def head_loss(target, root, prec1=False, joint_with=None):
+    old = _HeadLoss.active
+    ok = (root is not None and isinstance(target, torch.Tensor) and target.is_cuda and target.dtype == torch.int64 and target.dim() == 1
+          and target.is_contiguous())
+    _HeadLoss.active = (target, root, bool(prec1), joint_with) if ok else None
+    try:
+        yield
+    finally:
+        _HeadLoss.active = old
+
+
+def _head_loss_ok(x, weight, hl):
+    return (x.is_cuda and x.dtype in (torch.float32, torch.bfloat16) and hl[0].shape[0] == x.shape[0] and hl[0].device == x.device
+            and 0 < x.shape[0] * weight.shape[0] <= ops.CE_MAX_ELEMS and weight.is_contiguous())
+
+
 class _CEFn(torch.autograd.Function):
 
     @staticmethod
-    def forward(ctx, logits, target):
+    def forward(ctx, logits, target, rec=None):
+        ctx.rec = None
+        if rec is not None:
+            ctx.rec = rec
+            ctx.save_for_backward(logits, target)
+            return rec["loss"].reshape(())
         loss, dlogits = ops.cross_entropy(logits, target)
         ctx.save_for_backward(dlogits)
         return loss.reshape(())
 
     @staticmethod
     def backward(ctx, g):
-        (dlogits,) = ctx.saved_tensors
+        rec, ctx.rec = ctx.rec, None
+        if rec is not None:
+            logits, target = ctx.saved_tensors
+            if g.data_ptr() == rec["root_ptr"] and g.numel() == 1 and g.dtype == torch.float32:
+                rec["taken"] = True
+                return rec["dlogits"], None, None
+            _, dlogits = ops.cross_entropy(logits, target)
+        else:
+            (dlogits,) = ctx.saved_tensors
         if g.data_ptr() == ops.one(g.device).data_ptr():
-            return dlogits, None
-        return dlogits * g, None
+            return dlogits, None, None
+        return dlogits * g, None, None
 
 
 _FUSED_CE = os.environ.get("AFAN_FUSED_CE", "1") != "0"
@@ -986,8 +1041,12 @@
     def ce(out, y):
         if (out.is_cuda and out.dtype == torch.float32 and out.dim() == 2 and out.is_contiguous() and y.dtype == torch.int64
                 and y.dim() == 1 and 0 < out.numel() <= ops.CE_MAX_ELEMS):
-            return _CEFn.apply(out, y)
+            rec = getattr(out, "_afan_ce", None)
+            if rec is not None and not (rec["target"] is y and rec["logits_mark"] == (out.data_ptr(), out._version)):
+                rec = None
+            return _CEFn.apply(out, y, rec)
         return criterion(out, y)
+    ce._afan_fused = True
     return ce
 
 
diff --git a/cv_a-fan_amd/train_step.py b/cv_a-fan_amd/train_step.py
--- a/cv_a-fan_amd/train_step.py
+++ b/cv_a-fan_amd/train_step.py
@@ -162,6 +162,24 @@
 
     def last_diag(self):
         return None
+
+
+def _pgd_start(fm):
+    return fm if (ops.HEAD_CE or fm.dtype == torch.float32) else fm.float()
+
+
+def _observables(out_clean, out_adv, loss_clean, loss_adv, target):
+    rc, ra = getattr(out_clean, "_afan_ce", None), getattr(out_adv, "_afan_ce", None)
+    with torch.no_grad():
+        if ra is not None and ra.get("loss_joint") is not None and ra["target"] is target:
+            loss = ra["loss_joint"]
+        else:
+            loss = (loss_adv + loss_clean) / 2
+        if rc is not None and rc.get("prec1") is not None and rc["target"] is target:
+            prec1 = rc["prec1"]
+        else:
+            prec1 = (out_clean.argmax(dim=1) == target).float().sum() * (100.0 / target.shape[0])
+    return loss, prec1
 
 
 def _cut_chunks(arena, n_chunks):
@@ -278,22 +296,23 @@
         with ops.bn_running_updates(2):
             fm_clean = m(inp, end_point=idx, start_point=0)
         xin = fm_clean.detach().requires_grad_(True)
-        with ops.record_bn_updates() as clean_bn:
+        hroot = half if getattr(crit, "_afan_fused", False) else None
+        with ops.record_bn_updates() as clean_bn, resnet_s.head_loss(target, hroot, prec1=True):
             output_clean = m(xin, end_point=ln, start_point=idx)
         loss_clean = crit(output_clean, target)
         with resnet_s.stash_wgrad():
             torch.autograd.backward(loss_clean, grad_tensors=half)
         g0 = xin.grad
-        feature_map = fm_clean.detach()
-        feature_map = feature_map.float() if feature_map.dtype != torch.float32 else feature_map
-        feature_map_adv = PGD(feature_map, self.criterion, y=target, model=m, steps=self.steps,
+        feature_map_adv = PGD(_pgd_start(fm_clean.detach()), self.criterion, y=target, model=m, steps=self.steps,
                               gamma=(self.gamma / 255), start_idx=idx, layer_number=ln, eps=(self.eps / 255),
                               randinit=False, clip=self.clip, with_norms=True, grad0=g0)
+        feature_map = feature_map_adv._afan_x32
         l2, linf = last_norms()
         adv_in = getattr(feature_map_adv, "_afan_shadow", None)
         if adv_in is None:
             adv_in = feature_map_adv.detach()
-        output_adv = m(adv_in, end_point=ln, start_point=idx)
+        with resnet_s.head_loss(target, hroot, joint_with=loss_clean.detach().reshape(1)):
+            output_adv = m(adv_in, end_point=ln, start_point=idx)
         loss_adv = crit(output_adv, target)
         torch.autograd.backward(loss_adv, grad_tensors=half)
         resnet_s.flush_wgrad(m)
@@ -301,9 +320,7 @@
         if overlap_allreduce:
             self.reducer.begin()
         fm_clean.backward(g0)
-        with torch.no_grad():
-            loss = (loss_adv + loss_clean) / 2
-            prec1 = (output_clean.argmax(dim=1) == target).float().sum() * (100.0 / target.shape[0])
+        loss, prec1 = _observables(output_clean, output_adv, loss_clean, loss_adv, target)
         return {"loss": loss.detach(), "loss_adv": loss_adv.detach(), "loss_clean": loss_clean.detach(),
                 "prec1": prec1, "l2": l2, "linf": linf, "x_adv": feature_map_adv.detach(),
                 "feature_map": feature_map, "out_clean": output_clean.detach()}
@@ -345,7 +362,8 @@
         with ops.bn_running_updates(2):
             fm_clean = m(inp, end_point=idx, start_point=0)
         xin = fm_clean.detach().requires_grad_(True)
-        with ops.record_bn_updates() as clean_bn:
+        hroot = half if getattr(crit, "_afan_fused", False) else None
+        with ops.record_bn_updates() as clean_bn, resnet_s.head_loss(target, hroot, prec1=True):
             c_ins, c_outs = run_segments(xin)
         loss_clean = crit(c_outs[-1], target)
         with resnet_s.stash_wgrad():
@@ -353,16 +371,16 @@
             for k in range(len(segs) - 2, -1, -1):
                 c_outs[k].backward(c_ins[k + 1].grad)
         g0 = xin.grad
-        feature_map = fm_clean.detach()
-        feature_map = feature_map.float() if feature_map.dtype != torch.float32 else feature_map
-        feature_map_adv = PGD(feature_map, self.criterion, y=target, model=m, steps=self.steps,
+        feature_map_adv = PGD(_pgd_start(fm_clean.detach()), self.criterion, y=target, model=m, steps=self.steps,
                               gamma=(self.gamma / 255), start_idx=idx, layer_number=ln, eps=(self.eps / 255),
                               randinit=False, clip=self.clip, with_norms=True, grad0=g0)
+        feature_map = feature_map_adv._afan_x32
         l2, linf = last_norms()
         adv_in = getattr(feature_map_adv, "_afan_shadow", None)
         if adv_in is None:
             adv_in = feature_map_adv.detach()
-        a_ins, a_outs = run_segments(adv_in)
+        with resnet_s.head_loss(target, hroot, joint_with=loss_clean.detach().reshape(1)):
+            a_ins, a_outs = run_segments(adv_in)
         loss_adv = crit(a_outs[-1], target)
         torch.autograd.backward(loss_adv, grad_tensors=half)
         resnet_s.flush_wgrad(m.sequential_model[segs[-1][0]:segs[-1][1]])
@@ -377,9 +395,7 @@
             if len(segs) == 1:
                 clean_bn.replay()
             fm_clean.backward(g0)
-        with torch.no_grad():
-            loss = (loss_adv + loss_clean) / 2
-            prec1 = (c_outs[-1].argmax(dim=1) == target).float().sum() * (100.0 / target.shape[0])
+        loss, prec1 = _observables(c_outs[-1], a_outs[-1], loss_clean, loss_adv, target)
         out.update({"loss": loss.detach(), "loss_adv": loss_adv.detach(), "loss_clean": loss_clean.detach(),
                     "prec1": prec1, "l2": l2, "linf": linf, "x_adv": feature_map_adv.detach(),
                     "feature_map": feature_map, "out_clean": c_outs[-1].detach()})
@@ -405,12 +421,12 @@
         else:
             with torch.no_grad():
                 feature_map = m(inp, end_point=idx, start_point=0)
-        feature_map = feature_map.float() if feature_map.dtype != torch.float32 else feature_map
         from . import resnet_s as _rsb
         with _rsb.bn_branch(m, "adv"):
-            feature_map_adv = PGD(feature_map, self.criterion, y=target, model=m, steps=self.steps,
+            feature_map_adv = PGD(_pgd_start(feature_map), self.criterion, y=target, model=m, steps=self.steps,
                                   gamma=(self.gamma / 255), start_idx=idx, layer_number=ln, eps=(self.eps / 255),
                                   randinit=self.randinit, clip=self.clip, with_norms=True)
+        feature_map = feature_map_adv._afan_x32
         l2, linf = last_norms()
         adv_in = getattr(feature_map_adv, "_afan_shadow", None)
         if adv_in is None:
diff --git a/include/afan_hip.h b/include/afan_hip.h
--- a/include/afan_hip.h
+++ b/include/afan_hip.h
@@ -313,6 +313,10 @@
 int afan_cross_entropy(const float* logits, const int64_t* target, int64_t n, int64_t k, float* loss, float* dlogits,
                        afan_stream_t stream);
 
+int afan_head_ce(const void* x, int dtype, int64_t n, int64_t c, int64_t hw, const float* weight, const float* bias, int64_t k,
+                 const int64_t* target, const float* root, float* pooled, float* logits, float* dlogits, void* dx, void* rows,
+                 void* ticket, float* loss, float* prec1, const float* loss_other, float* loss_joint, afan_stream_t stream);
+
 int afan_transpose_weights(const void* src_arena, void* dst_arena, const int64_t* desc_dev, int n_desc,
                            int64_t total_tiles, afan_stream_t stream);
 
@@ -328,6 +332,8 @@
 
 int afan_cast_bf16(const float* src, uint16_t* dst, int64_t n, afan_stream_t stream);
 int afan_pgd_init(const void* x, int dtype, float* x32, float* x_adv, uint16_t* shadow, int64_t n, afan_stream_t stream);
+int afan_pgd_init_step(const void* x, int dtype, const void* grad, int grad_dtype, float* x32, float* x_adv, uint16_t* shadow,
+                       int64_t n, float gamma, float eps, int clip, afan_stream_t stream);
 int afan_normalize_nchw(const float* x, void* y, int out_dtype, int out_layout, int64_t n, int64_t c, int64_t hw,
                         const float* mean, const float* std, afan_stream_t stream);
 
```

Result: no change. 33590 images/sec (median of 6 runs) (+0.9%).
